# kwohlfahrt/collision

Measured on AMD Instinct MI355X. Metric: M spheres/sec end-to-end (bounds->Morton->radix sort->LBVH->refit->traversal), higher is better.
Workload: dtype f32 coords / u32 keys+ids; 1 GPU; BASELINE config 2: 1000000 uniform-random spheres, r=0.001, f32, RandomState(4), pair capacity 131072; spheres_total=1000000, group_size=256, parallelism=single

## Files before the change

collision_amd/csrc/bvh.hip:

```cpp
#include "col_common.h"
#include <math.h>

namespace {

constexpr u32 END = 0xFFFFFFFFu;

template <typename T> struct BTypes;
template <> struct BTypes<float> {
    typedef float4 V4;
    typedef uint32_t Bits;
    struct alignas(4) V3 { float x, y, z; };
};
template <> struct BTypes<double> {
    typedef double4 V4;
    typedef uint64_t Bits;
    struct alignas(8) V3 { double x, y, z; };
};

template <typename T> __device__ __forceinline__ u32 link_load(const T *bounds, uint64_t row) {
    typedef typename BTypes<T>::Bits Bits;
    return (u32) reinterpret_cast<const Bits *>(bounds)[row * 4 + 3];
}
template <typename T> __device__ __forceinline__ void link_store(T *bounds, uint64_t row, u32 v) {
    typedef typename BTypes<T>::Bits Bits;
// ... 923 lines not shown
    if (g_traverse_variant & 16) mode |= 8;
    if (g_traverse_variant & 256) mode |= 1;
    if (g_traverse_variant & 512) mode |= 2;
    if (g_traverse_variant & 16777216) mode |= 2048;
    if (g_traverse_variant & 33554432) mode |= 4096;
    constexpr int MAX_DEV = 16;
    static u64 *spread_dev[MAX_DEV] = {nullptr};
    static u32 *dyn_sched_dev[MAX_DEV] = {nullptr};
    int dev = 0;
    if (g_traverse_variant & (1024 | 8192)) {
        COL_HIP(hipGetDevice(&dev));
        if (dev < 0 || dev >= MAX_DEV) return COL_EINVAL;
    }
    u64 *&spread = spread_dev[dev];
    if (g_traverse_variant & 1024) {
        if (!spread && hipMalloc((void **)&spread, 8192 * 32 * 4) != hipSuccess) return COL_EINVAL;
        mode |= 16;
    }
    const bool off32 = (2ull * n - 1) * 8 * sizeof(T) < (1ull << 32) && !(g_traverse_variant & 64) && ((uintptr_t)bounds & 63) == 0;
    u32 *&dyn_sched = dyn_sched_dev[dev];
    if ((g_traverse_variant & 8192) && !sched && !st && !(mode & (32 | 64))) {
        if (!dyn_sched && hipMalloc((void **)&dyn_sched, 64) != hipSuccess) return COL_EINVAL;
        COL_HIP(hipMemsetAsync(dyn_sched, 0, 64, s));
        sched = dyn_sched;
    }
    if (sched && !st && !(g_traverse_variant & (16384 | 1 | 2 | 4 | 128 | 1024))) {
        mode |= 256;
        if (g_traverse_variant & 4194304) mode |= 128;
        if (g_traverse_variant & 8388608) mode |= 1024;
        if ((n <= COL_SPLIT_UNITS_UPTO || (g_traverse_variant & 65536)) && !(g_traverse_variant & 131072)) mode |= 512;
        if (off32 && (g_traverse_variant & 4096)) k_traverse<T, false, false, 1, false, true><<<g, t, 0, s>>>(pairs, counter, capacity, bd, n, (u64 *)sched, mode, NoGhost{}, n_dev, (g_traverse_variant & 2097152) ? nullptr : walk_order);
        else if (off32) k_traverse<T, false, false, 1><<<g, t, 0, s>>>(pairs, counter, capacity, bd, n, (u64 *)sched, mode, NoGhost{}, n_dev, (g_traverse_variant & 2097152) ? nullptr : walk_order);
        else k_traverse<T, false, false, 0><<<g, t, 0, s>>>(pairs, counter, capacity, bd, n, (u64 *)sched, mode, NoGhost{}, n_dev, (g_traverse_variant & 2097152) ? nullptr : walk_order);
        COL_LAUNCH_OK();
        return COL_OK;
    }
    if ((g_traverse_variant & 255) == 1) k_traverse_lane<T><<<g, t, 0, s>>>(pairs, counter, capacity, bd, n, 0);
    else if (st) k_traverse<T, true, false, 0><<<g, t, 0, s>>>(pairs, counter, capacity, bd, n, st, mode);
    else if (g_traverse_variant & 2) k_traverse<T, false, true, 0><<<g, t, 0, s>>>(pairs, counter, capacity, bd, n, st, mode);
    else if (off32 && (g_traverse_variant & 128)) k_traverse<T, false, false, 2><<<g, t, 0, s>>>(pairs, counter, capacity, bd, n, st, mode);
    else if (off32 && (g_traverse_variant & 4096)) k_traverse<T, false, false, 1, false, true><<<g, t, 0, s>>>(pairs, counter, capacity, bd, n, st, mode, NoGhost{}, n_dev);
    else if (off32) k_traverse<T, false, false, 1><<<g, t, 0, s>>>(pairs, counter, capacity, bd, n, (g_traverse_variant & 1024) ? spread : st, mode, NoGhost{}, n_dev);
    else k_traverse<T, false, false, 0><<<g, t, 0, s>>>(pairs, counter, capacity, bd, n, st, mode, NoGhost{}, n_dev);
    COL_LAUNCH_OK();
    return COL_OK;
}

__global__ __launch_bounds__(256) void k_pairs_compact(u32 *__restrict__ pairs, const ChunkHdr *__restrict__ hdr, u32 nholes) {
    __shared__ u32 s_start[512], s_len[512];
    __shared__ u32 s_low[513], s_fill[513];
    __shared__ u32 s_b[513], s_e[513];
    if (hdr->overflow) return;
    const u32 A = hdr->A, T = hdr->T, tid = threadIdx.x;
    if (A == T) return;
    __shared__ unsigned long long s_bits[1024];
    __shared__ u32 s_wpre[1024];
    __shared__ u32 s_ws2[4];
    for (u32 i = tid; i < 1024; i += 256) s_bits[i] = 0;
    for (u32 i = tid; i < 513; i += 256) { if (i < 512) { s_start[i] = A; s_len[i] = 0; } }
    __syncthreads();
    uint2 mine[2];
#pragma unroll
    for (int u = 0; u < 2; u++) {
        const u32 i = tid + 256 * u;
        mine[u] = i < nholes ? hdr->holes[i] : make_uint2(0u, 0u);
        if (mine[u].y) {
            const u32 c = mine[u].x / (u32)CHUNK_PAIRS;
            atomicOr(&s_bits[c >> 6], 1ull << (c & 63u));
        }
    }
    __syncthreads();
    {
        u32 pc[4], sum = 0;
#pragma unroll
        for (int u = 0; u < 4; u++) { pc[u] = (u32)__popcll(s_bits[4 * tid + u]); sum += pc[u]; }
        u32 total;
        u32 run = block_excl_scan<256>(sum, s_ws2, &total);
#pragma unroll
        for (int u = 0; u < 4; u++) { s_wpre[4 * tid + u] = run; run += pc[u]; }
    }
    __syncthreads();
#pragma unroll
    for (int u = 0; u < 2; u++)
        if (mine[u].y) {
            const u32 c = mine[u].x / (u32)CHUNK_PAIRS;
            const u32 rank = s_wpre[c >> 6] + (u32)__popcll(s_bits[c >> 6] & ((1ull << (c & 63u)) - 1ull));
            s_start[rank] = mine[u].x; s_len[rank] = mine[u].y;
        }
    __syncthreads();
    {
        __shared__ u32 s_ws[4];
        u32 lowc[2], highc[2], bb[2], ee[2];
#pragma unroll
        for (int u = 0; u < 2; u++) {
            const u32 i = 2 * tid + u;
            const u32 st = s_start[i], ln = s_len[i];
            bb[u] = ln ? (st > T ? st : T) : A;
            ee[u] = ln ? (st + ln > T ? st + ln : T) : A;
            lowc[u] = ln ? (st >= T ? 0u : (st + ln <= T ? ln : T - st)) : 0u;
            highc[u] = ee[u] - bb[u];
        }
        u32 total_low, total_high;
        const u32 plow = block_excl_scan<256>(lowc[0] + lowc[1], s_ws, &total_low);
        const u32 phigh = block_excl_scan<256>(highc[0] + highc[1], s_ws, &total_high);
#pragma unroll
        for (int u = 0; u < 2; u++) {
            const u32 i = 2 * tid + u;
            const u32 lo_before = plow + (u ? lowc[0] : 0u), hi_before = phigh + (u ? highc[0] : 0u);
            s_low[i] = lo_before;
            s_b[i] = bb[u]; s_e[i] = ee[u];
            s_fill[i] = (bb[u] - T) - hi_before;
        }
        if (tid == 0) {
            s_low[512] = total_low;
            s_fill[512] = (A - T) - total_high;
            s_b[512] = A; s_e[512] = A;
        }
    }
    __syncthreads();
    const u32 moves = s_low[512];
    constexpr int MV = 4;
    const u32 stride = gridDim.x * 256;
    for (u32 k0 = blockIdx.x * 256 + tid; k0 < moves; k0 += MV * stride) {
        u32 kk[MV], lo1[MV], lo2[MV];
#pragma unroll
        for (int u = 0; u < MV; u++) { kk[u] = min(k0 + u * stride, moves - 1u); lo1[u] = 0; lo2[u] = 0; }
#pragma unroll
        for (u32 step = 256; step; step >>= 1) {
#pragma unroll
            for (int u = 0; u < MV; u++) {
                if (s_low[lo1[u] + step] <= kk[u]) lo1[u] += step;
                if (s_fill[lo2[u] + step] <= kk[u]) lo2[u] += step;
            }
        }
        uint2 pr[MV];
        u32 dst[MV];
#pragma unroll
        for (int u = 0; u < MV; u++) {
            dst[u] = s_start[lo1[u]] + (kk[u] - s_low[lo1[u]]);
            const u32 src = kk[u] < s_fill[0] ? T + kk[u] : s_e[lo2[u]] + (kk[u] - s_fill[lo2[u]]);
            pr[u] = *reinterpret_cast<const uint2 *>(pairs + 2ull * src);
        }
#pragma unroll
        for (int u = 0; u < MV; u++)
            if (k0 + u * stride < moves) *reinterpret_cast<uint2 *>(pairs + 2ull * dst[u]) = pr[u];
    }
}

template <typename T>
int launch_traverse_chunked(void *stream, uint32_t *pairs, uint32_t *counter, uint32_t capacity, const void *bounds,
                            uint32_t n, void *scratch, const uint32_t *n_dev = nullptr, uint32_t *walk_order = nullptr,
                            bool hdr_cleared = false) {
    const bool split = (n <= COL_SPLIT_UNITS_UPTO || (g_traverse_variant & 65536)) && !(g_traverse_variant & 131072);
    const int dyn = (g_traverse_variant & 16384) ? 0 : (split ? 256 | 512 : 256) | ((g_traverse_variant & 4194304) ? 128 : 0) | ((g_traverse_variant & 8388608) ? 1024 : 0);
    const u32 npackets = (n + 63) / 64;
    u32 blocks = (u32)col_ceil_div(npackets, TW);
    if (blocks > 512) blocks = 512;
    dim3 g(blocks), t(TT);
    hipStream_t s = col_stream(stream);
    const T *bd = (const T *)bounds;
    ChunkHdr *hdr = (ChunkHdr *)scratch;
    if (!hdr_cleared) COL_HIP(hipMemsetAsync(hdr, 0, 64, s));
    k_traverse<T, false, false, 1><<<g, t, 0, s>>>(pairs, counter, capacity, bd, n, (u64 *)hdr, 32 | dyn, NoGhost{}, n_dev,
                                                   (dyn & 256) && !(g_traverse_variant & 2097152) ? walk_order : nullptr);
    COL_LAUNCH_OK();
    if (capacity) {
        k_pairs_compact<<<dim3(512), dim3(256), 0, s>>>(pairs, hdr, blocks);
        COL_LAUNCH_OK();
        k_traverse<T, false, false, 1><<<g, t, 0, s>>>(pairs, counter, capacity, bd, n, (u64 *)hdr, 64, NoGhost{}, n_dev);
        COL_LAUNCH_OK();
    }
    return COL_OK;
}

template <typename T>
int launch_ghost(void *stream, uint32_t *pairs, uint32_t *counter, uint32_t capacity, const void *bounds, uint32_t n,
                 const GhostArgs &ga, uint32_t max_ghosts, const uint32_t *n_dev) {
    const u32 npackets = (max_ghosts + 63) / 64;
    u32 blocks = (u32)col_ceil_div(npackets, TW);
    if (blocks > 512) blocks = 512;
    if (blocks == 0) return COL_OK;
    dim3 g(blocks), t(TT);
    hipStream_t s = col_stream(stream);
    const T *bd = (const T *)bounds;
    const bool off32 = (2ull * n - 1) * 8 * sizeof(T) < (1ull << 32) && !(g_traverse_variant & 64) && ((uintptr_t)bounds & 63) == 0;
    if (off32) k_traverse<T, false, false, 1, true><<<g, t, 0, s>>>(pairs, counter, capacity, bd, n, nullptr, 0, ga, n_dev);
    else k_traverse<T, false, false, 0, true><<<g, t, 0, s>>>(pairs, counter, capacity, bd, n, nullptr, 0, ga, n_dev);
    COL_LAUNCH_OK();
    return COL_OK;
}

}

extern "C" int col_traverse_ghost_packets(void *stream, uint32_t *pairs, uint32_t *counter, uint32_t capacity, const void *bounds,
                                          uint32_t n, int coord_bytes, const uint32_t *rec, const uint32_t *order,
                                          const uint32_t *count, uint32_t max_ghosts, const uint32_t *local_gids,
                                          const uint32_t *n_dev) {
    if (n == 0 || max_ghosts == 0) return COL_OK;
    const GhostArgs ga = {rec, order, count, local_gids};
    if (coord_bytes == 4) return launch_ghost<float>(stream, pairs, counter, capacity, bounds, n, ga, max_ghosts, n_dev);
    if (coord_bytes == 8) return launch_ghost<double>(stream, pairs, counter, capacity, bounds, n, ga, max_ghosts, n_dev);
    return COL_EINVAL;
}

extern "C" {

void col_debug_traverse(int variant) { g_traverse_variant = variant; }
int col_debug_walk_profile(uint32_t *out, uint32_t npackets) {
    if (npackets > COL_PROF_PACKETS) return COL_EINVAL;
    COL_HIP(hipDeviceSynchronize());
    COL_HIP(hipMemcpyFromSymbol(out, HIP_SYMBOL(g_walk_prof), 16ull * npackets));
    return COL_OK;
}

int col_bvh_build(void *stream, const uint32_t *codes, const uint32_t *ids, col_node *nodes, void *bounds,
                  uint32_t n, int coord_bytes) {
    if (n == 0) return COL_OK;
    if (n >= 0x80000000u) return COL_EINVAL;
    dim3 grid((unsigned)col_ceil_div(n, 256)), block(256);
    if (coord_bytes == 4) k_build<float><<<grid, block, 0, col_stream(stream)>>>(codes, ids, nodes, (float *)bounds, n);
    else if (coord_bytes == 8) k_build<double><<<grid, block, 0, col_stream(stream)>>>(codes, ids, nodes, (double *)bounds, n);
    else return COL_EINVAL;
    COL_LAUNCH_OK();
    return COL_OK;
}

int col_bvh_refit(void *stream, void *bounds, uint32_t *flags, const void *coords, const void *radii,
                  const col_node *nodes, uint32_t n, int coord_bytes) {
    if (n == 0) return COL_OK;
    if (coord_bytes != 4 && coord_bytes != 8) return COL_EINVAL;
    hipStream_t s = col_stream(stream);
    dim3 leaves((unsigned)col_ceil_div(n, 256)), inner((unsigned)col_ceil_div(n > 1 ? n - 1 : 1, 256)),
        all((unsigned)col_ceil_div(2ull * n - 1, 256)), block(256);
    int rounds = 16;
    for (uint32_t m = n; m > 1; m >>= 1) rounds++;
    uint32_t *progress = (n > (uint32_t)rounds + 1) ? flags + (n - 1) : nullptr;
    if (coord_bytes == 4) {
        k_refit_leaves<float><<<leaves, block, 0, s>>>((float *)bounds, flags, (const float *)coords, (const float *)radii, nodes, n);
        if (n > 1) {
            for (int r = 1; r <= rounds; r++) k_refit_sweep<float><<<inner, block, 0, s>>>((float *)bounds, flags, nodes, n, (u32)r, progress);
            k_refit_finish<float><<<all, block, 0, s>>>((float *)bounds, flags, nodes, n, progress ? progress + rounds : nullptr);
        }
    } else {
        k_refit_leaves<double><<<leaves, block, 0, s>>>((double *)bounds, flags, (const double *)coords, (const double *)radii, nodes, n);
        if (n > 1) {
            for (int r = 1; r <= rounds; r++) k_refit_sweep<double><<<inner, block, 0, s>>>((double *)bounds, flags, nodes, n, (u32)r, progress);
            k_refit_finish<double><<<all, block, 0, s>>>((double *)bounds, flags, nodes, n, progress ? progress + rounds : nullptr);
        }
    }
    COL_LAUNCH_OK();
    return COL_OK;
}

int col_traverse(void *stream, uint32_t *pairs, uint32_t *counter, uint32_t capacity, const col_node *nodes,
                 const void *bounds, uint32_t n, int coord_bytes) {
    (void)nodes;
    if (n < 2) return COL_OK;
    if (capacity > 0 && !pairs) return COL_EINVAL;
    if (coord_bytes == 4) return launch_traverse<float>(stream, pairs, counter, capacity, bounds, n, nullptr, 0);
    if (coord_bytes == 8) return launch_traverse<double>(stream, pairs, counter, capacity, bounds, n, nullptr, 0);
    return COL_EINVAL;
}

size_t col_traverse_chunked_scratch_bytes(void) { return sizeof(ChunkHdr); }

static int traverse_chunked_dev(void *stream, uint32_t *pairs, uint32_t *counter, uint32_t capacity, const col_node *nodes,
                                const void *bounds, uint32_t n, int coord_bytes, void *scratch, const uint32_t *n_dev,
                                uint32_t *walk_order = nullptr, bool hdr_cleared = false);
int col_traverse_chunked(void *stream, uint32_t *pairs, uint32_t *counter, uint32_t capacity, const col_node *nodes,
                         const void *bounds, uint32_t n, int coord_bytes, void *scratch) {
    return traverse_chunked_dev(stream, pairs, counter, capacity, nodes, bounds, n, coord_bytes, scratch, nullptr);
}
static int traverse_chunked_dev(void *stream, uint32_t *pairs, uint32_t *counter, uint32_t capacity, const col_node *nodes,
                                const void *bounds, uint32_t n, int coord_bytes, void *scratch, const uint32_t *n_dev,
                                uint32_t *walk_order, bool hdr_cleared) {
    const bool off32 = (coord_bytes == 4 || coord_bytes == 8) && (2ull * n - 1) * 8 * (unsigned)coord_bytes < (1ull << 32) &&
                       ((uintptr_t)bounds & 63) == 0;
    if (!off32 || !scratch || (g_traverse_variant & ~(16384 | 32768 | 65536 | 131072 | 2097152 | 4194304 | 8388608)))
    {
        if (n < 2) return COL_OK;
        if (capacity > 0 && !pairs) return COL_EINVAL;
        if (coord_bytes == 4) return launch_traverse<float>(stream, pairs, counter, capacity, bounds, n, nullptr, 0, nullptr, n_dev);
        if (coord_bytes == 8) return launch_traverse<double>(stream, pairs, counter, capacity, bounds, n, nullptr, 0, nullptr, n_dev);
        return COL_EINVAL;
    }
    if (n < 2) return COL_OK;
    if (capacity > 0 && !pairs) return COL_EINVAL;
    if (coord_bytes == 8) return launch_traverse_chunked<double>(stream, pairs, counter, capacity, bounds, n, scratch, n_dev, walk_order, hdr_cleared);
    return launch_traverse_chunked<float>(stream, pairs, counter, capacity, bounds, n, scratch, n_dev, walk_order, hdr_cleared);
}

int col_traverse_stats(void *stream, uint32_t *pairs, uint32_t *counter, uint32_t capacity, const void *bounds,
                       uint32_t n, int coord_bytes, uint64_t *stats, int mode) {
    if (n < 2) return COL_OK;
    if (coord_bytes == 4) return launch_traverse<float>(stream, pairs, counter, capacity, bounds, n, stats, mode);
    if (coord_bytes == 8) return launch_traverse<double>(stream, pairs, counter, capacity, bounds, n, stats, mode);
    return COL_EINVAL;
}

size_t col_collide_scratch_bytes(uint32_t n, uint32_t padded, int coord_bytes) {
    return 256  + col_reduce_scratch_bytes(coord_bytes == 8 ? COL_F64 : COL_F32, 4) +
           col_radix_scratch_bytes(padded, 4, 4) + col_lbvh_scratch_bytes(n, coord_bytes) +
           (size_t)n * 4 * coord_bytes  + sizeof(ChunkHdr) + 256  + 1024 +
           8 * ((size_t)n / 64 + 1) + 256 ;
}

int col_collide(void *stream, const void *coords, const void *radii, uint32_t n, uint32_t padded, int coord_bytes,
                uint32_t *codes0, uint32_t *codes1, uint32_t *ids0, uint32_t *ids1, col_node *nodes, void *bounds,
                uint32_t *flags, void *scratch, uint32_t *counter, uint32_t *pairs, uint32_t capacity) {
    return col_collide_plan(stream, coords, radii, n, padded, coord_bytes, codes0, codes1, ids0, ids1, nodes, bounds, flags,
                            scratch, counter, pairs, capacity, COL_SORT_LSD, nullptr);
}

int col_collide_plan(void *stream, const void *coords, const void *radii, uint32_t n, uint32_t padded, int coord_bytes,
                     uint32_t *codes0, uint32_t *codes1, uint32_t *ids0, uint32_t *ids1, col_node *nodes, void *bounds,
                     uint32_t *flags, void *scratch, uint32_t *counter, uint32_t *pairs, uint32_t capacity,
                     int sort_plan, uint32_t *oversize) {
    return col_collide_plan_partials(stream, coords, radii, n, padded, coord_bytes, codes0, codes1, ids0, ids1, nodes, bounds,
                                     flags, scratch, counter, pairs, capacity, sort_plan, oversize, nullptr, 0);
}

int col_collide_plan_partials(void *stream, const void *coords, const void *radii, uint32_t n, uint32_t padded, int coord_bytes,
                              uint32_t *codes0, uint32_t *codes1, uint32_t *ids0, uint32_t *ids1, col_node *nodes, void *bounds,
                              uint32_t *flags, void *scratch, uint32_t *counter, uint32_t *pairs, uint32_t capacity,
                              int sort_plan, uint32_t *oversize, const void *partials, uint32_t parts) {
    return col_collide_plan_dev(stream, coords, radii, n, padded, coord_bytes, codes0, codes1, ids0, ids1, nodes, bounds, flags, scratch,
                                counter, pairs, capacity, sort_plan, oversize, partials, parts, nullptr);
}

int col_collide_plan_dev(void *stream, const void *coords, const void *radii, uint32_t n, uint32_t padded, int coord_bytes,
                         uint32_t *codes0, uint32_t *codes1, uint32_t *ids0, uint32_t *ids1, col_node *nodes, void *bounds,
                         uint32_t *flags, void *scratch, uint32_t *counter, uint32_t *pairs, uint32_t capacity,
                         int sort_plan, uint32_t *oversize, const void *partials, uint32_t parts, const uint32_t *n_dev) {
    if (coord_bytes != 4 && coord_bytes != 8) return COL_EINVAL;
    if (n_dev && !partials) return COL_EINVAL;
    if (partials && (parts == 0 || parts > COL_MINMAX_PARTS)) return COL_EINVAL;
    if (padded < n || (capacity > 0 && !pairs)) return COL_EINVAL;
    if (!scratch) return COL_ENOSCRATCH;
    if (col_radix_tile_override_active()) return COL_EINVAL;
    hipStream_t s = col_stream(stream);
    if (n == 0) {
        COL_HIP(hipMemsetAsync(counter, 0, sizeof(uint32_t), s));
        return COL_OK;
    }
    (void)flags;
    char *p = (char *)scratch;
    void *range = p;           p += 256;
    void *red_scratch = p;     p += col_reduce_scratch_bytes(coord_bytes == 8 ? COL_F64 : COL_F32, 4);
    p = (char *)(((uintptr_t)p + 255) & ~(uintptr_t)255);
    void *sort_scratch = p;    p += col_radix_scratch_bytes(padded, 4, 4);
    p = (char *)(((uintptr_t)p + 255) & ~(uintptr_t)255);
    void *lbvh_scratch = p;    p += col_lbvh_scratch_bytes(n, coord_bytes);
    p = (char *)(((uintptr_t)p + 255) & ~(uintptr_t)255);
    void *packed = p;          p += (size_t)n * 4 * coord_bytes;
    p = (char *)(((uintptr_t)p + 255) & ~(uintptr_t)255);
    void *chunk_hdr = p;
    const bool chunked = (sort_plan & COL_TRAVERSE_CHUNKED) != 0;
    sort_plan &= 1;
    uint32_t *publish = oversize ? oversize + 2 : nullptr;
    int rc;
    uint32_t *report_word = nullptr;
    const uint32_t tile = col_radix_tile(padded, 4, 4);
    if (tile == 1024 || tile == 4096 || tile == 8192) {
        const bool msd = sort_plan == COL_SORT_MSD && padded <= COL_MSD_MAX_N;
        if (!partials) {
            if ((rc = col_minmax4_stage1(stream, coords, n, coord_bytes, red_scratch, &parts))) return rc;
            partials = red_scratch;
        }
        if ((rc = col_morton_tile(stream, coords, radii, partials, parts, n, padded, coord_bytes, codes0, ids0, packed,
                                  counter, (uint32_t *)sort_scratch, tile, (uint32_t)col_ceil_div(padded, tile), msd ? 22 : 0,
                                  publish, n_dev))) return rc;
        if (msd) rc = col_radix_sort_msd_dev(stream, codes0, codes1, ids0, ids1, padded, sort_scratch, oversize, n_dev);
        else rc = col_radix_sort_ex(stream, codes0, codes1, ids0, ids1, padded, 4, 4, sort_scratch, 0, 1);
        if (rc) return rc;
        if (!msd && oversize && padded <= COL_MSD_MAX_N) report_word = oversize + 1;
    } else {
        if (n_dev) return COL_EINVAL;
        if ((rc = col_reduce(stream, coords, n, coord_bytes == 8 ? COL_F64 : COL_F32, 4, COL_OP_MINMAX, red_scratch, range))) return rc;
        if ((rc = col_morton_ex(stream, coords, radii, range, n, padded, coord_bytes, codes0, ids0, packed, counter, publish))) return rc;
        if ((rc = col_radix_sort(stream, codes0, codes1, ids0, ids1, padded, 4, 4, sort_scratch, 0))) return rc;
    }
    uint32_t *sched = (!chunked && (n >= COL_DYNAMIC_PACKETS_FROM || (g_traverse_variant & 32768))) ? (uint32_t *)((char *)chunk_hdr + sizeof(ChunkHdr)) : nullptr;
    const int order_mode = chunked || col_lbvh_order_forced() ? 1 : 0;
    uint32_t *walk_order = n > 256 && (chunked || (sched && (n <= COL_DEAL_MAX_N || order_mode))) ? (uint32_t *)((char *)chunk_hdr + sizeof(ChunkHdr) + 256) : nullptr;
    if ((rc = col_lbvh_ex(stream, codes1, ids1, coords, radii, packed, nodes, bounds, lbvh_scratch, n, coord_bytes,
                          chunked ? (uint32_t *)chunk_hdr : sched, n_dev, walk_order, order_mode, chunked ? 16u : 8u, report_word, padded))) return rc;
    if (chunked) return traverse_chunked_dev(stream, pairs, counter, capacity, nodes, bounds, n, coord_bytes, chunk_hdr, n_dev, walk_order, true);
    if (n < 2) return COL_OK;
    if (coord_bytes == 4) return launch_traverse<float>(stream, pairs, counter, capacity, bounds, n, nullptr, 0, sched, n_dev, walk_order);
    return launch_traverse<double>(stream, pairs, counter, capacity, bounds, n, nullptr, 0, sched, n_dev, walk_order);
}

}
```

collision_amd/csrc/col_common.h:

```cpp
#pragma once
#include <hip/hip_runtime.h>
#include <stdint.h>
#include "../../include/collision_hip.h"
#include "../../include/collision_hip_debug.h"

#define COL_WAVE 64

#define COL_HIP(expr)                                  \
    do {                                               \
        hipError_t e_ = (expr);                        \
        if (e_ != hipSuccess) return (int)e_;          \
    } while (0)

#define COL_LAUNCH_OK()                                \
    do {                                               \
        hipError_t e_ = hipGetLastError();             \
        if (e_ != hipSuccess) return (int)e_;          \
    } while (0)

extern "C" int col_morton_ex(void *stream, const void *coords, const void *radii, const void *range, uint32_t n,
                             uint32_t padded, int coord_bytes, uint32_t *codes, uint32_t *ids, void *packed,
                             uint32_t *zero_word, uint32_t *publish);
extern "C" int col_lbvh_ex(void *stream, const uint32_t *codes, const uint32_t *ids, const void *coords, const void *radii,
                           const void *packed, col_node *nodes, void *bounds, void *scratch, uint32_t n, int coord_bytes,
                           uint32_t *zero8,
                           const uint32_t *n_dev,
                           uint32_t *walk_order,
                           int order_mode,
                           uint32_t nzero = 8,
                           uint32_t *report_word = nullptr,
                           uint32_t report_n = 0);
extern "C" int col_lbvh_order_forced(void);
extern "C" int col_radix_sort_msd_dev(void *stream, const uint32_t *keys, uint32_t *keys_out, const uint32_t *vals, uint32_t *vals_out,
                                      uint64_t n, void *scratch, uint32_t *oversize, const uint32_t *n_real_dev);

#define COL_MINMAX_PARTS 256
#define COL_REGION_BOXES 8
#define COL_MSD_SMALL_N 1900000u
#define COL_MSD_MAX_N 4050000u
extern "C" int col_minmax4_stage1(void *stream, const void *rows, uint64_t n, int coord_bytes, void *partials, uint32_t *parts);
extern "C" int col_minmax4_stage1_dev(void *stream, const void *rows, const uint32_t *n_dev, uint32_t n_max, int coord_bytes,
                                      void *partials, uint32_t *parts);
extern "C" int col_morton_tile(void *stream, const void *coords, const void *radii, const void *partials, uint32_t parts,
                               uint32_t n, uint32_t padded, int coord_bytes, uint32_t *codes, uint32_t *ids, void *packed,
                               uint32_t *zero_word, uint32_t *hist0, uint32_t tile, uint32_t nblocks, int hist_shift,
                               uint32_t *publish, const uint32_t *n_dev);
extern "C" int col_radix_sort_ex(void *stream, const void *keys, void *keys_out, const void *vals, void *vals_out,
                                 uint64_t n, int key_bytes, int val_bytes, void *scratch, int copy_back, int have_hist0);

extern "C" int col_traverse_ghost_packets(void *stream, uint32_t *pairs, uint32_t *counter, uint32_t capacity, const void *bounds,
                                          uint32_t n, int coord_bytes, const uint32_t *rec, const uint32_t *order,
                                          const uint32_t *count, uint32_t max_ghosts, const uint32_t *local_gids,
                                          const uint32_t *n_dev);
extern "C" int col_radix_sort_low_passes(void *stream, const uint32_t *keys, uint32_t *keys_out, const uint32_t *vals,
                                         uint32_t *vals_out, uint64_t n, void *scratch, int passes);
extern "C" int col_radix_bucket_report(void *stream, const uint32_t *sorted_codes, uint64_t n, uint32_t *word);
extern "C" int col_radix_tile_override_active(void);

static inline hipStream_t col_stream(void *s) { return (hipStream_t)s; }

static inline uint64_t col_ceil_div(uint64_t a, uint64_t b) { return (a + b - 1) / b; }

#ifdef __HIPCC__
typedef unsigned long long u64;
typedef unsigned int u32;
__device__ __forceinline__ void col_bucket_report_block(const u32 *__restrict__ sorted, u32 n, u32 *word, u32 *s_start) {
    const u32 d = threadIdx.x;
    const u32 want = d << 22;
    u32 lo = 0, hi = n;
    while (lo < hi) {
        const u32 mid = lo + ((hi - lo) >> 1);
        if (sorted[mid] < want) lo = mid + 1; else hi = mid;
    }
    s_start[d] = lo;
    if (d == 0) {
        u32 l2 = 0, h2 = n;
        while (l2 < h2) {
            const u32 mid = l2 + ((h2 - l2) >> 1);
            if (sorted[mid] < (1u << 30)) l2 = mid + 1; else h2 = mid;
        }
        s_start[256] = l2;
    }
    __syncthreads();
    u32 cnt = s_start[d + 1] - s_start[d];
#pragma unroll
    for (int o = COL_WAVE / 2; o > 0; o >>= 1) cnt = max(cnt, (u32)__shfl_xor((int)cnt, o, COL_WAVE));
    __syncthreads();
    if ((d & 63u) == 0) s_start[d >> 6] = cnt;
    __syncthreads();
    if (d == 0) {
        const u32 m = max(max(s_start[0], s_start[1]), max(s_start[2], s_start[3]));
        __hip_atomic_store(word, 0x80000000u | min(m, 0x7FFFFFFFu), __ATOMIC_RELAXED, __HIP_MEMORY_SCOPE_SYSTEM);
    }
}

__device__ __forceinline__ u32 lane_id() { return __lane_id(); }

__device__ __forceinline__ u32 count_of(u32 n, const u32 *__restrict__ n_dev) { return n_dev ? min(n, *n_dev) : n; }

__device__ __forceinline__ u32 mbcnt(u64 mask) {
    return __builtin_amdgcn_mbcnt_hi((u32)(mask >> 32), __builtin_amdgcn_mbcnt_lo((u32)mask, 0u));
}

__device__ __forceinline__ u32 wave_incl_scan(u32 v) {
    const u32 lane = lane_id();
#pragma unroll
    for (int o = 1; o < COL_WAVE; o <<= 1) {
        u32 t = __shfl_up(v, o, COL_WAVE);
        if (lane >= (u32)o) v += t;
    }
    return v;
}

__device__ __forceinline__ u32 wave_sum(u32 v) {
#pragma unroll
    for (int o = COL_WAVE / 2; o > 0; o >>= 1) v += __shfl_xor(v, o, COL_WAVE);
    return v;
}

template <int NT>
__device__ __forceinline__ u32 block_excl_scan(u32 v, u32 *warp_sums, u32 *total) {
    constexpr int NW = NT / COL_WAVE;
    const u32 lane = lane_id(), w = threadIdx.x / COL_WAVE;
    u32 incl = wave_incl_scan(v);
    if (lane == COL_WAVE - 1) warp_sums[w] = incl;
    __syncthreads();
    u32 base = 0, tot = 0;
#pragma unroll
    for (int i = 0; i < NW; i++) {
        u32 s = warp_sums[i];
        if ((u32)i < w) base += s;
        tot += s;
    }
    __syncthreads();
    *total = tot;
    return base + incl - v;
}
#define COL_LEAF_BLOCK 16u
#define COL_LINK_MARK 0x80000000u
#define COL_LEAF_BLOCK_MAX_N (1u << 27)
__device__ __forceinline__ u32 block_link(u32 lo, u32 hi) { return COL_LINK_MARK | (lo << 4) | (hi - lo); }
__device__ __forceinline__ u32 descend_link(u32 down, u32 leaf_start, bool marks) {
    return (marks && (down & COL_LINK_MARK)) ? leaf_start + ((down >> 4) & 0x7FFFFFFu) : down;
}
#define COL_DEAL_MAX_N 1310720u
#define COL_TRAV_WAVES 16u
#define COL_TRAV_FIRST_BATCHES 64
__device__ __forceinline__ void xcd_packet_range(u32 npackets, u32 x, u32 &p_lo, u32 &p_end) {
    const u32 ng = (npackets + COL_TRAV_WAVES - 1) / COL_TRAV_WAVES;
    p_lo = (u32)(((u64)ng * x) >> 3) * COL_TRAV_WAVES;
    p_end = min((u32)(((u64)ng * (x + 1)) >> 3) * COL_TRAV_WAVES, npackets);
}
__device__ __forceinline__ u32 expand_bits(u32 v) {
    v = (v * 0x00010001u) & 0xFF0000FFu;
    v = (v * 0x00000101u) & 0x0F00F00Fu;
    v = (v * 0x00000011u) & 0xC30C30C3u;
    v = (v * 0x00000005u) & 0x49249249u;
    return v;
}
template <typename T> __device__ __forceinline__ T tmax(T a, T b);
template <> __device__ __forceinline__ float tmax(float a, float b) { return fmaxf(a, b); }
template <> __device__ __forceinline__ double tmax(double a, double b) { return fmax(a, b); }
template <typename T> __device__ __forceinline__ T tmin(T a, T b);
template <> __device__ __forceinline__ float tmin(float a, float b) { return fminf(a, b); }
template <> __device__ __forceinline__ double tmin(double a, double b) { return fmin(a, b); }
template <typename T>
__device__ __forceinline__ u32 quantize(T p, T mn, T mx) {
    T t = (p - mn) / (mx - mn);
    t = t * (T)1023;
    t = tmin(tmax(t, (T)0), (T)1023);
    return (u32)t;
}
template <typename T>
__device__ __forceinline__ u32 morton30(T x, T y, T z, T mnx, T mny, T mnz, T mxx, T mxy, T mxz) {
    return (expand_bits(quantize(x, mnx, mxx)) << 2) + (expand_bits(quantize(y, mny, mxy)) << 1) +
           expand_bits(quantize(z, mnz, mxz));
}
#endif
```

collision_amd/csrc/lbvh.hip:

```cpp
#include "col_common.h"
#include <math.h>

namespace {

constexpr u32 END = 0xFFFFFFFFu;
constexpr int C = 256;
constexpr int LV = 9;

template <typename T> struct BT;
template <> struct BT<float> { typedef float4 V4; typedef uint32_t Bits; };
template <> struct BT<double> { typedef double4 V4; typedef uint64_t Bits; };

template <typename T> struct Box { T lo[3], hi[3]; };

template <typename T> __device__ __forceinline__ Box<T> box_empty() {
    Box<T> b;
#pragma unroll
    for (int a = 0; a < 3; a++) { b.lo[a] = (T)INFINITY; b.hi[a] = -(T)INFINITY; }
    return b;
}
__device__ __forceinline__ float hw_min(float a, float b) { float r; asm("v_min_f32 %0, %1, %2" : "=v"(r) : "v"(a), "v"(b)); return r; }
__device__ __forceinline__ float hw_max(float a, float b) { float r; asm("v_max_f32 %0, %1, %2" : "=v"(r) : "v"(a), "v"(b)); return r; }
__device__ __forceinline__ double hw_min(double a, double b) { double r; asm("v_min_f64 %0, %1, %2" : "=v"(r) : "v"(a), "v"(b)); return r; }
__device__ __forceinline__ double hw_max(double a, double b) { double r; asm("v_max_f64 %0, %1, %2" : "=v"(r) : "v"(a), "v"(b)); return r; }
// ... 462 lines not shown
        leaf.lo[0] = c.x - r; leaf.lo[1] = c.y - r; leaf.lo[2] = c.z - r;
        leaf.hi[0] = c.x + r; leaf.hi[1] = c.y + r; leaf.hi[2] = c.z + r;
        lds.leaf[0][tid] = c.x; lds.leaf[1][tid] = c.y; lds.leaf[2][tid] = c.z; lds.leaf[3][tid] = r;
    }

    Box<T> pre = leaf, suf = leaf;
    if constexpr (DPP_SCAN) {
        wave_prefix_union(pre);
        wave_suffix_union(suf);
    } else {
#pragma unroll
        for (int o = 1; o < COL_WAVE; o <<= 1) {
            const Box<T> up = box_shfl_up(pre, o), dn = box_shfl_down(suf, o);
            if (lane >= o) box_merge(pre, up);
            if (lane + o < COL_WAVE) box_merge(suf, dn);
        }
    }
    if (lane == COL_WAVE - 1) { for (int k = 0; k < 3; k++) { lds.wave_tot[0][w][k] = pre.lo[k]; lds.wave_tot[0][w][3 + k] = pre.hi[k]; } }
    if (lane == 0) { for (int k = 0; k < 3; k++) { lds.wave_tot[1][w][k] = suf.lo[k]; lds.wave_tot[1][w][3 + k] = suf.hi[k]; } }
    __syncthreads();
    for (int ww = 0; ww < C / COL_WAVE; ww++) {
        Box<T> t;
        for (int k = 0; k < 3; k++) { t.lo[k] = lds.wave_tot[ww < w ? 0 : 1][ww][k]; t.hi[k] = lds.wave_tot[ww < w ? 0 : 1][ww][3 + k]; }
        if (ww < w) box_merge(pre, t);
        if (ww > w) box_merge(suf, t);
    }

    if (valid) {
        LeafTail tail = {p, id};
        *reinterpret_cast<LeafTail *>(&nodes[leaf_start + p].right_edge) = tail;
        u32 skip_leaf = END;
        if (p + 1 < n) {
            if constexpr (FAST_DELTA && sizeof(I) == 4) {
                const u32 k = p + 1;
                if (k + 1 >= n) skip_leaf = (n - 1) + k;
                else if (tid + 1 < C) skip_leaf = lds.adj[tid + 2] > d_next ? k : (n - 1) + k;
                else skip_leaf = right_child_at(codes, k);
            } else skip_leaf = right_child_at(codes, p + 1);
        }
        record_store(bounds, (uint64_t)leaf_start + p, leaf, skip_leaf, id);
    }
    if (tid == 0)
        box_store(tab1, ((uint64_t)(chunk / C) * LV + 0) * C + (chunk % C), suf);
    if (p == n - 1 && n > (u32)C) box_store(partial, p, pre);
    if constexpr (CLIMB) {
        if (valid) {
            int l = tid, r = tid, my_split = 0;
            bool is_leaf = true;
            Box<T> box = leaf;
            for (;;) {
                const int dl = lds.adj[l], dr = lds.adj[r + 1];
                const bool right = dr > dl;
                if (!is_leaf) {
                    const int node = right ? r : l;
                    soa_put(lds.node, node, box);
                    lds.oe[node] = (unsigned char)(right ? l : r);
                    lds.split[node] = (unsigned char)my_split;
                }
                const int g = right ? r : l - 1;
                if ((dl & dr) < 0 || g < 0 || g >= C - 1) break;
                asm volatile("" ::: "memory");
                const u32 place = 16u * ((u32)g & 1u);
                const u32 old = (__hip_atomic_fetch_or(&lds.flags[g >> 1], ((u32)(right ? l : r) + 1u) << place, __ATOMIC_RELAXED, __HIP_MEMORY_SCOPE_WORKGROUP) >> place) & 0xFFFFu;
                asm volatile("" ::: "memory");
                if (old == 0) break;
                const int far = (int)old - 1;
                Box<T> sib;
                if (right) { sib = far == g + 1 ? leaf_get(lds.leaf, g + 1) : soa_get(lds.node, g + 1); r = far; }
                else { sib = far == g ? leaf_get(lds.leaf, g) : soa_get(lds.node, g); l = far; }
                box_merge(box, sib);
                my_split = g;
                is_leaf = false;
            }
        }
        __syncthreads();
    }
    auto search = [&](u32 t, u32 &j, u32 &gamma) {
        const u32 i = c0 + t, ci = codes.win[HALO + t];
        int dir, delta_min;
        if constexpr (FAST_DELTA && sizeof(I) == 4) {
            const int dn = lds.adj[t + 1], dp = lds.adj[t];
            dir = dn > dp ? 1 : -1;
            delta_min = min(dn, dp);
        } else {
            dir = delta(codes, i, ci, (I)i + 1) > delta(codes, i, ci, (I)i - 1) ? 1 : -1;
            delta_min = delta(codes, i, ci, (I)i - dir);
        }
        I len_max = 2;
        while (delta(codes, i, ci, (I)i + dir * len_max) > delta_min) len_max *= 2;
        I len = 0;
        for (I t2 = len_max / 2; t2 > 0; t2 /= 2)
            if (delta(codes, i, ci, (I)i + dir * (len + t2)) > delta_min) len += t2;
        j = (u32)((I)i + dir * len);
        const int delta_node = delta(codes, i, ci, (I)j);
        I s = 0, t2 = len;
        do {
            t2 = (t2 + 1) / 2;
            if (delta(codes, i, ci, (I)i + dir * (s + t2)) > delta_node) s += t2;
        } while (t2 > 1);
        gamma = dir > 0 ? (u32)(i + s) : (u32)(i - s - 1);
    };
    auto node_out = [&](u32 t, u32 j, u32 gamma, u32 &skip, u32 &child_a) {
        const u32 i = c0 + t;
        const u32 lo = min(i, j), hi = max(i, j);
        const bool a_leaf = lo == gamma, b_leaf = hi == gamma + 1;
        child_a = a_leaf ? leaf_start + gamma : gamma;
        const u32 child_b = b_leaf ? leaf_start + gamma + 1 : gamma + 1;
        InnerTail tail = {hi, child_a, child_b};
        *reinterpret_cast<InnerTail *>(&nodes[i].right_edge) = tail;
        if (!(dbg & 2)) { nodes[child_a].parent = i; nodes[child_b].parent = i; }
        other_end[i] = j;
        skip = END;
        if (hi + 1 < n) {
            if constexpr (FAST_DELTA && sizeof(I) == 4) {
                const u32 k = hi + 1;
                if (k + 1 >= n) skip = (n - 1) + k;
                else if (hi >= c0 && k < c0 + (u32)C) skip = lds.adj[k - c0 + 1] > lds.adj[hi - c0 + 1] ? k : (n - 1) + k;
                else {
                    const u32 ck = gcodes[k], cm = gcodes[k - 1u], cp = gcodes[k + 1u];
                    const u32 d_fwd = min(ffbh_raw(ck ^ cp), 32u + ffbh_raw(k ^ (k + 1u))), d_bwd = min(ffbh_raw(ck ^ cm), 32u + ffbh_raw(k ^ (k - 1u)));
                    skip = d_fwd > d_bwd ? k : (n - 1) + k;
                }
            } else skip = right_child_at(codes, hi + 1);
        }
    };
    auto record_out = [&](u32 i, u32 j, u32 skip, u32 child_a, const Box<T> &box) {
        const u32 lo = min(i, j), hi = max(i, j);
        u32 down = child_a;
        if (hi - lo < COL_LEAF_BLOCK && n <= COL_LEAF_BLOCK_MAX_N && block_k > (T)0) {
            const Box<T> first = leaf_get(lds.leaf, (int)(lo - c0));
            bool dense = true;
#pragma unroll
            for (int k = 0; k < 3; k++) dense = dense && (box.hi[k] - box.lo[k]) <= block_k * (first.hi[k] - first.lo[k]);
            if (dense) down = block_link(lo, hi);
        }
        record_store(bounds, (uint64_t)i, box, skip, down);
    };
    auto crossing_out = [&](u32 i, int dir) {
        box_store(partial, i, dir > 0 ? suf : pre);
        const u32 slot = atomicAdd(&lds.ncross, 1u);
        cross[(uint64_t)chunk * CROSS_CAP + (slot < CROSS_CAP - 1 ? slot : CROSS_CAP - 1)] = slot < CROSS_CAP - 1 ? i : CROSS_DENSE;
    };
    if constexpr (CLIMB) {
        const bool inner = p < leaf_start;
        const bool named = inner && lds.oe[tid] != (unsigned char)tid;
        u32 skip, child_a;
        if (named) {
            const u32 j = c0 + lds.oe[tid];
            node_out((u32)tid, j, c0 + lds.split[tid], skip, child_a);
            record_out(p, j, skip, child_a, soa_get(lds.node, tid));
        } else if (inner) crossing_out(p, d_next > d_prev ? 1 : -1);
        const u64 todo = __builtin_amdgcn_ballot_w64(inner && !named);
        if (todo == 0) return;
        const u32 cnt = (u32)__builtin_popcountll(todo);
        const u32 lpn_log = cnt <= 1 ? 6u : cnt <= 2 ? 5u : cnt <= 4 ? 4u : 3u, lpn = 1u << lpn_log, groups = 64u >> lpn_log;
        const u32 g = (u32)lane >> lpn_log, sub = (u32)lane & (lpn - 1u);
        auto group_count = [&](bool yes) -> I {
            u64 m = __builtin_amdgcn_ballot_w64(yes) >> (g << lpn_log);
            if (lpn < 64u) m &= (1ull << lpn) - 1ull;
            return (I)__builtin_popcountll(m);
        };
        for (u32 base = 0; base < cnt; base += groups) {
            const bool on = base + g < cnt;
            u64 m = todo;
            for (u32 b = 0; b < base + g && on; b++) m &= m - 1ull;
            const u32 t = on ? (u32)w * COL_WAVE + (u32)__builtin_ctzll(m) : (u32)tid;
            const u32 i = c0 + t, ci = codes.win[HALO + t];
            const int dn = lds.adj[t + 1], dp = lds.adj[t];
            const int dir = dn > dp ? 1 : -1, delta_min = min(dn, dp);
            auto yes_at = [&](I x, int thr) -> bool {
                const I jk = (I)i + dir * x;
                const bool inb = on && x > 0 && (u32)jk < n;
                const u32 o = (u32)(jk - codes.w0);
                const bool inwin = o < (u32)WIN;
                u32 cj;
                if (__builtin_amdgcn_ballot_w64(inb && !inwin) == 0) cj = codes.win[inwin ? o : 0u];
                else cj = inb ? (inwin ? codes.win[o] : gcodes[jk]) : 0u;
                const u32 d = min(ffbh_raw(ci ^ cj), 32u + ffbh_raw(i ^ (u32)jk));
                return inb && (int)d > thr;
            };
            I hi = 2;
            {
                bool more = on;
                int e0 = 1;
                while (__builtin_amdgcn_ballot_w64(more)) {
                    const int e = e0 + (int)sub;
                    const I x = (more && e < 31 && (1u << e) <= n) ? (I)(1u << e) : (I)0;
                    const I yes = group_count(yes_at(x, delta_min));
                    if (more) {
                        hi = (I)(1u << (e0 + yes));
                        more = yes == (I)lpn && e0 + (int)lpn < 31;
                        e0 += (int)lpn;
                    }
                }
            }
            auto run_end = [&](I lo, I hi, int thr) -> I {
                while (__builtin_amdgcn_ballot_w64(on && hi - lo > 1)) {
                    const bool act = on && hi - lo > 1;
                    const I step = (hi - lo + (I)lpn) / ((I)lpn + 1);
                    const I x = lo + ((I)sub + 1) * step;
                    const I yes = group_count(yes_at(act && x < hi ? x : (I)0, thr));
                    if (act) { lo += yes * step; hi = min(hi, lo + step); }
                }
                return lo;
            };
            const I len = run_end(hi / 2, hi, delta_min);
            const u32 j = (u32)((I)i + dir * len);
            const int delta_node = delta(codes, i, ci, (I)j);
            const I s = run_end((I)0, len, delta_node);
            const u32 gamma = dir > 0 ? (u32)(i + s) : (u32)(i - s - 1);
            if (on && sub == 0) {
                node_out(t, j, gamma, skip, child_a);
                links_store(bounds, (uint64_t)i, skip, child_a);
            }
        }
        return;
    }
    if (p >= leaf_start || (dbg & 4)) return;
    u32 j = 0, gamma = 0, skip, child_a;
    search((u32)tid, j, gamma);
    const u32 i = p;
    const u32 lo = min(i, j), hi = max(i, j);
    node_out((u32)tid, j, gamma, skip, child_a);
    if (dbg & 8) return;
    if (lo >= c0 && hi < c0 + C) {
        const bool a_leaf = lo == gamma, b_leaf = hi == gamma + 1;
        const int la = (int)(gamma - c0), lb = la + 1;
        Box<T> box;
        const int fa = a_leaf ? C : la, fb = b_leaf ? C : lb;
        for (bool done = false; !done;) {
            const u32 ra = __hip_atomic_load(&lds.flags[fa], __ATOMIC_RELAXED, __HIP_MEMORY_SCOPE_WORKGROUP);
            const u32 rb = __hip_atomic_load(&lds.flags[fb], __ATOMIC_RELAXED, __HIP_MEMORY_SCOPE_WORKGROUP);
            if (ra & rb) {
                __builtin_amdgcn_fence(__ATOMIC_ACQUIRE, "workgroup");
                box = a_leaf ? leaf_get(lds.leaf, la) : soa_get(lds.node, la);
                box_merge(box, b_leaf ? leaf_get(lds.leaf, lb) : soa_get(lds.node, lb));
                soa_put(lds.node, tid, box);
                __hip_atomic_store(&lds.flags[tid], 1u, __ATOMIC_RELEASE, __HIP_MEMORY_SCOPE_WORKGROUP);
                done = true;
            }
        }
        record_out(i, j, skip, child_a, box);
    } else {
        links_store(bounds, (uint64_t)i, skip, child_a);
        crossing_out(i, j > i ? 1 : -1);
    }
}

template <typename T>
__global__ __launch_bounds__(C) void k_group(T *__restrict__ tab, u32 count, T *__restrict__ next, u32 n_bound, const u32 *__restrict__ n_dev,
                                             int level) {
    if (n_dev) {
        u32 c = count_of(n_bound, n_dev);
        for (int k = 0; k <= level; k++) c = (c + C - 1) / C;
        count = min(count, c);
    }
    __shared__ Table<T> t;
    const int tid = threadIdx.x;
    const u32 g = blockIdx.x;
    const u32 e = g * C + tid;
    const uint64_t base = (uint64_t)g * LV * C;
    Box<T> b = e < count ? box_load(tab, base + tid) : box_empty<T>();
    if (e >= count) box_store(tab, base + tid, b);
    tab_put(t, 0, tid, b);
    tab_build(t, tid);
    for (int l = 1; l < LV; l++) box_store(tab, base + (uint64_t)l * C + tid, tab_get(t, l, tid));
    if (tid == 0 && next) box_store(next, ((uint64_t)(g / C) * LV + 0) * C + (g % C), tab_get(t, LV - 1, 0));
}

struct Tabs { void *t[3]; };

constexpr u32 LIN = 32;

template <typename T>
__device__ __forceinline__ void cross_node(T *__restrict__ bounds, const u32 *__restrict__ other_end, const T *__restrict__ partial,
                                           const Tabs &tabs, u32 i, int lin) {
    const u32 j = other_end[i];
    const u32 first = min(i, j), last = max(i, j);
    int64_t a = first / C, b = last / C;
    if (a == b) return;
    Box<T> box = box_load(partial, first);
    box_merge(box, box_load(partial, last));
    a += 1; b -= 1;
    for (int h = 0; h < 3 && a <= b; h++) {
        const T *tab = (const T *)tabs.t[h];
        if (h == lin) {
            for (int64_t e = a; e <= b; e++) box_merge(box, box_load(tab, (uint64_t)e));
            break;
        }
        const int64_t ga = a / C, gb = b / C;
        if (ga == gb) {
            box_merge(box, gtab_query(tab, (uint64_t)ga, (int)(a % C), (int)(b % C)));
            break;
        }
        box_merge(box, gtab_query(tab, (uint64_t)ga, (int)(a % C), C - 1));
        box_merge(box, gtab_query(tab, (uint64_t)gb, 0, (int)(b % C)));
        a = ga + 1; b = gb - 1;
    }
    T *row = bounds + 8ull * i;
    row[0] = box.lo[0]; row[1] = box.lo[1]; row[2] = box.lo[2];
    row[4] = box.hi[0]; row[5] = box.hi[1]; row[6] = box.hi[2];
}

template <typename T>
__global__ __launch_bounds__(256) void k_cross(T *__restrict__ bounds, const u32 *__restrict__ other_end,
                                               const T *__restrict__ partial, const u32 *__restrict__ cross, Tabs tabs, u32 n,
                                               u32 nchunks, int lin, u32 *__restrict__ zero8, const u32 *__restrict__ n_dev,
                                               u32 *__restrict__ walk_order, u32 cross_blocks, int order_mode, u32 nzero) {
    const u32 n_bound = n;
    if (n_dev) { n = count_of(n, n_dev); nchunks = min(nchunks, (n + (u32)C - 1) / (u32)C); }
    if (blockIdx.x >= cross_blocks) {
        order_packets(blockIdx.x - cross_blocks, n, n_bound, walk_order, order_mode);
        return;
    }
    const u32 t = blockIdx.x * 256 + threadIdx.x;
    if (zero8 && t < nzero) zero8[t] = 0;
    const u32 chunk = t / CROSS_CAP, slot = t % CROSS_CAP;
    if (chunk >= nchunks) return;
    if (cross[(uint64_t)chunk * CROSS_CAP + CROSS_CAP - 1] == CROSS_DENSE) {
        for (u32 k = slot; k < (u32)C; k += CROSS_CAP) {
            const u32 i = chunk * C + k;
            if (i + 1 < n) cross_node(bounds, other_end, partial, tabs, i, lin);
        }
        return;
    }
    const u32 i = cross[(uint64_t)chunk * CROSS_CAP + slot];
    if (i != END) cross_node(bounds, other_end, partial, tabs, i, lin);
}

int g_dbg = 0;
float g_block_k = 3.0f;
inline size_t align256(size_t x) { return (x + 255) & ~(size_t)255; }

struct Layout {
    size_t other_end, partial, cross, tab[3], total;
    u32 count[3];
};

Layout layout(uint32_t n, int coord_bytes) {
    Layout L;
    const size_t entry = 8 * (size_t)coord_bytes;
    size_t off = 0;
    L.other_end = off; off += align256((size_t)n * 4);
    L.partial = off;   off += align256((size_t)n * entry);
    u32 cnt = (u32)col_ceil_div(n, C);
    L.cross = off;     off += align256((size_t)cnt * CROSS_CAP * 4);
    for (int h = 0; h < 3; h++) {
        L.count[h] = cnt;
        const size_t groups = col_ceil_div(cnt, C);
        L.tab[h] = off; off += align256(groups * LV * C * entry);
        cnt = (u32)groups;
    }
    L.total = off;
    return L;
}

template <typename T>
int run(hipStream_t s, const u32 *codes, const u32 *ids, const T *coords, const T *radii, const T *packed,
        col_node *nodes, T *bounds, char *scratch, u32 n, u32 *zero8, const u32 *n_dev, u32 *walk_order, int order_mode,
        u32 nzero, u32 *report_word, u32 report_n) {
    const Layout L = layout(n, sizeof(T));
    u32 *other_end = (u32 *)(scratch + L.other_end);
    T *partial = (T *)(scratch + L.partial);
    u32 *cross = (u32 *)(scratch + L.cross);
    Tabs tabs;
    for (int h = 0; h < 3; h++) tabs.t[h] = scratch + L.tab[h];
    const u32 nchunks = L.count[0];
    bool ordered_by_chunk = false;
    if (g_dbg & ~(1024 | 2048 | 4096 | 8192 | 16384))
        k_chunk<T, true, int64_t><<<dim3(nchunks), dim3(C), 0, s>>>(codes, ids, coords, radii, packed, nodes, bounds, other_end, partial, cross,
                                                                    (T *)tabs.t[0], n, (T)g_block_k, n_dev, ChunkDiagOn{g_dbg & ~(1024 | 2048 | 4096 | 8192 | 16384)});
    else if (n < (1u << 30) && (g_dbg & 8192))
        k_chunk<T, false, int32_t, true, true><<<dim3(nchunks), dim3(C), 0, s>>>(codes, ids, coords, radii, packed, nodes, bounds, other_end, partial, cross,
                                                                                 (T *)tabs.t[0], n, (T)g_block_k, n_dev, ChunkDiagOff{});
    else if (n < (1u << 30) && !(g_dbg & 1024) && !((g_dbg & 2048) && sizeof(T) == 8))
    {
        k_chunk<T, false, int32_t, true, true, true><<<dim3(nchunks + (walk_order ? 8u * COL_ORDER_SLICES : 0u) + (report_word ? 1u : 0u)), dim3(C), (g_dbg & 16384) ? 24576 : 0, s>>>(
            codes, ids, coords, radii, packed, nodes, bounds, other_end, partial, cross, (T *)tabs.t[0], n, (T)g_block_k, n_dev, ChunkDiagOff{}, walk_order, order_mode,
            report_word, report_n);
        ordered_by_chunk = true;
        report_word = nullptr;
    }
    else if (n < (1u << 30) && !(g_dbg & 1024))
        k_chunk<T, false, int32_t, false, true><<<dim3(nchunks), dim3(C), 0, s>>>(codes, ids, coords, radii, packed, nodes, bounds, other_end, partial, cross,
                                                                                  (T *)tabs.t[0], n, (T)g_block_k, n_dev, ChunkDiagOff{});
    else if (n < (1u << 30))
        k_chunk<T, false, int32_t><<<dim3(nchunks), dim3(C), 0, s>>>(codes, ids, coords, radii, packed, nodes, bounds, other_end, partial, cross,
                                                                     (T *)tabs.t[0], n, (T)g_block_k, n_dev, ChunkDiagOff{});
    else
        k_chunk<T, false, int64_t><<<dim3(nchunks), dim3(C), 0, s>>>(codes, ids, coords, radii, packed, nodes, bounds, other_end, partial, cross,
                                                                     (T *)tabs.t[0], n, (T)g_block_k, n_dev, ChunkDiagOff{});
    COL_LAUNCH_OK();
    if (report_word) {
        const int rc = col_radix_bucket_report((void *)s, codes, report_n, report_word);
        if (rc) return rc;
    }
    if (nchunks < 2) {
        if (zero8) COL_HIP(hipMemsetAsync(zero8, 0, nzero * sizeof(u32), s));
        return COL_OK;
    }
    int lin = -1;
    for (int h = 0; h < 3; h++) {
        if (h > 0 && L.count[h] <= LIN) { lin = h; break; }
        const u32 groups = (u32)col_ceil_div(L.count[h], C);
        k_group<T><<<dim3(groups), dim3(C), 0, s>>>((T *)tabs.t[h], L.count[h], h + 1 < 3 ? (T *)tabs.t[h + 1] : nullptr, n, n_dev, h);
        COL_LAUNCH_OK();
        if (groups < 2) break;
    }
    const unsigned cross_blocks = (unsigned)col_ceil_div((uint64_t)nchunks * CROSS_CAP, 256);
    k_cross<T><<<dim3(cross_blocks + (walk_order && !ordered_by_chunk ? 8u * COL_ORDER_SLICES : 0u)), dim3(256), 0, s>>>(bounds, other_end, partial, cross, tabs, n, nchunks, lin, zero8,
                                                                                                          n_dev, walk_order, cross_blocks, order_mode, nzero);
    COL_LAUNCH_OK();
    return COL_OK;
}

}

extern "C" {

void col_debug_lbvh(int mode) { g_dbg = mode; }
int col_lbvh_order_forced(void) { return (g_dbg & 4096) ? 1 : 0; }
void col_debug_leaf_blocks(float k) { g_block_k = k; }

size_t col_lbvh_scratch_bytes(uint32_t n, int coord_bytes) { return layout(n, coord_bytes).total + 256; }

int col_lbvh_ex(void *stream, const uint32_t *codes, const uint32_t *ids, const void *coords, const void *radii,
                const void *packed, col_node *nodes, void *bounds, void *scratch, uint32_t n, int coord_bytes, uint32_t *zero8,
                const uint32_t *n_dev, uint32_t *walk_order, int order_mode, uint32_t nzero, uint32_t *report_word, uint32_t report_n) {
    if (n == 0) return COL_OK;
    if (n >= 0x80000000u || nzero > 256u) return COL_EINVAL;
    if (!scratch) return COL_ENOSCRATCH;
    if (coord_bytes == 4)
        return run<float>(col_stream(stream), codes, ids, (const float *)coords, (const float *)radii, (const float *)packed,
                          nodes, (float *)bounds, (char *)scratch, n, zero8, n_dev, walk_order, order_mode, nzero, report_word, report_n);
    if (coord_bytes == 8)
        return run<double>(col_stream(stream), codes, ids, (const double *)coords, (const double *)radii,
                           (const double *)packed, nodes, (double *)bounds, (char *)scratch, n, zero8, n_dev, walk_order, order_mode, nzero, report_word, report_n);
    return COL_EINVAL;
}

int col_lbvh(void *stream, const uint32_t *codes, const uint32_t *ids, const void *coords, const void *radii,
             col_node *nodes, void *bounds, void *scratch, uint32_t n, int coord_bytes) {
    return col_lbvh_ex(stream, codes, ids, coords, radii, nullptr, nodes, bounds, scratch, n, coord_bytes, nullptr, nullptr, nullptr, 0);
}

}
```

collision_amd/csrc/morton.hip:

```cpp
#include "col_common.h"

namespace {


template <typename T> struct alignas(4 * sizeof(T)) Vec4 { T x, y, z, w; };
template <> struct alignas(16) Vec4<double> { double x, y, z, w; };

__device__ __forceinline__ void publish_count(u32 *publish, u32 count) {
    if (publish) __hip_atomic_store(publish, 0x80000000u | (count < 0x7FFFFFFFu ? count : 0x7FFFFFFFu), __ATOMIC_RELAXED, __HIP_MEMORY_SCOPE_SYSTEM);
}

template <typename T>
__global__ __launch_bounds__(256) void k_morton(const Vec4<T> *__restrict__ coords,
                                                 const Vec4<T> *__restrict__ range, u32 n, u32 padded,
                                                 u32 *__restrict__ codes, u32 *__restrict__ ids,
                                                 const T *__restrict__ radii, Vec4<T> *__restrict__ packed,
                                                 u32 *__restrict__ zero_word, u32 *publish) {
    const u32 i = blockIdx.x * 256 + threadIdx.x;
    if (i == 0 && zero_word) {
        publish_count(publish, *zero_word);
        *zero_word = 0;
    }
    if (i >= padded) return;
    u32 code = 0xFFFFFFFFu;
    if (i < n) {
        const Vec4<T> mn = range[0], mx = range[1];
        const Vec4<T> c = coords[i];
        if (packed) {
            Vec4<T> pr = c;
            pr.w = radii[i];
            packed[i] = pr;
        }
        code = (expand_bits(quantize(c.x, mn.x, mx.x)) << 2) + (expand_bits(quantize(c.y, mn.y, mx.y)) << 1) +
               expand_bits(quantize(c.z, mn.z, mx.z));
    }
    codes[i] = code;
    if (ids) ids[i] = i;
}

constexpr int MT_ROWS = 4;
template <typename T, int NT, int HALVES>
__global__ __launch_bounds__(NT) void k_morton_tile(const Vec4<T> *__restrict__ coords, const T *__restrict__ partials,
                                                     u32 parts, u32 n_bound, u32 padded, u32 *__restrict__ codes,
                                                     u32 *__restrict__ ids, const T *__restrict__ radii,
                                                     Vec4<T> *__restrict__ packed, u32 *__restrict__ zero_word,
                                                     u32 *__restrict__ hist0, u32 nblocks, int hist_shift, u32 *publish,
                                                     const u32 *__restrict__ n_dev) {
    constexpr int TILE = NT * MT_ROWS * HALVES, NW = NT / 64;
    const u32 n = count_of(n_bound, n_dev);
    __shared__ T s_fold[NW][8];
    __shared__ u32 s_hist[256];
    const u32 tid = threadIdx.x, lane = tid & 63u, w = tid >> 6;
    if (blockIdx.x == 0 && tid == 0 && zero_word) {
        publish_count(publish, *zero_word);
        *zero_word = 0;
    }
    if (tid < 256) s_hist[tid] = 0;
    Vec4<T> c[MT_ROWS];
    T rad[MT_ROWS];
#pragma unroll
    for (int k = 0; k < MT_ROWS; k++) {
        const u32 i = blockIdx.x * TILE + k * NT + tid;
        if (i < n) {
            c[k] = coords[i];
            if (packed) rad[k] = radii[i];
        }
    }
    T acc[8];
#pragma unroll
    for (int k = 0; k < 4; k++) { acc[k] = (T)INFINITY; acc[4 + k] = -(T)INFINITY; }
    for (u32 i = tid; i < parts; i += NT) {
        const T *q = partials + (size_t)i * 8;
#pragma unroll
        for (int k = 0; k < 4; k++) {
            acc[k] = q[k] < acc[k] ? q[k] : acc[k];
            acc[4 + k] = q[4 + k] > acc[4 + k] ? q[4 + k] : acc[4 + k];
        }
    }
#pragma unroll
    for (int o = 32; o > 0; o >>= 1) {
#pragma unroll
        for (int k = 0; k < 4; k++) {
            const T lo = __shfl_xor(acc[k], o, 64), hi = __shfl_xor(acc[4 + k], o, 64);
            acc[k] = lo < acc[k] ? lo : acc[k];
            acc[4 + k] = hi > acc[4 + k] ? hi : acc[4 + k];
        }
    }
    if (lane == 0) {
#pragma unroll
        for (int k = 0; k < 8; k++) s_fold[w][k] = acc[k];
    }
    __syncthreads();
    Vec4<T> mn, mx;
    {
        T r[8];
#pragma unroll
        for (int k = 0; k < 8; k++) r[k] = s_fold[0][k];
        for (int ww = 1; ww < NW; ww++) {
#pragma unroll
            for (int k = 0; k < 4; k++) {
                r[k] = s_fold[ww][k] < r[k] ? s_fold[ww][k] : r[k];
                r[4 + k] = s_fold[ww][4 + k] > r[4 + k] ? s_fold[ww][4 + k] : r[4 + k];
            }
        }
        mn.x = r[0]; mn.y = r[1]; mn.z = r[2]; mn.w = r[3];
        mx.x = r[4]; mx.y = r[5]; mx.z = r[6]; mx.w = r[7];
    }
#pragma unroll
    for (int h = 0; h < HALVES; h++) {
        if (h > 0) {
#pragma unroll
            for (int k = 0; k < MT_ROWS; k++) {
                const u32 i = blockIdx.x * TILE + (h * MT_ROWS + k) * NT + tid;
                if (i < n) {
                    c[k] = coords[i];
                    if (packed) rad[k] = radii[i];
                }
            }
        }
#pragma unroll
        for (int k = 0; k < MT_ROWS; k++) {
            const u32 i = blockIdx.x * TILE + (h * MT_ROWS + k) * NT + tid;
            if (i >= padded) continue;
            u32 code = 0xFFFFFFFFu;
            if (i < n) {
                if (packed) {
                    Vec4<T> pr = c[k];
                    pr.w = rad[k];
                    packed[i] = pr;
                }
                code = (expand_bits(quantize(c[k].x, mn.x, mx.x)) << 2) + (expand_bits(quantize(c[k].y, mn.y, mx.y)) << 1) +
                       expand_bits(quantize(c[k].z, mn.z, mx.z));
            }
            codes[i] = code;
            if (ids) ids[i] = i;
            atomicAdd(&s_hist[(code >> hist_shift) & 255u], 1u);
        }
    }
    __syncthreads();
    if (tid < 256) hist0[(uint64_t)tid * nblocks + blockIdx.x] = s_hist[tid];
}

template <typename T>
int launch_morton_tile(hipStream_t s, u32 tile, const void *coords, const void *radii, const void *partials, uint32_t parts,
                       uint32_t n, uint32_t padded, uint32_t *codes, uint32_t *ids, void *packed, uint32_t *zero_word,
                       uint32_t *hist0, uint32_t nblocks, int hist_shift, uint32_t *publish, const uint32_t *n_dev) {
    dim3 grid(nblocks);
    if (tile == 1024)
        k_morton_tile<T, 256, 1><<<grid, dim3(256), 0, s>>>((const Vec4<T> *)coords, (const T *)partials, parts, n, padded, codes, ids,
                                                             (const T *)radii, (Vec4<T> *)packed, zero_word, hist0, nblocks, hist_shift, publish, n_dev);
    else if (tile == 4096)
        k_morton_tile<T, 1024, 1><<<grid, dim3(1024), 0, s>>>((const Vec4<T> *)coords, (const T *)partials, parts, n, padded, codes, ids,
                                                               (const T *)radii, (Vec4<T> *)packed, zero_word, hist0, nblocks, hist_shift, publish, n_dev);
    else
        k_morton_tile<T, 1024, 2><<<grid, dim3(1024), 0, s>>>((const Vec4<T> *)coords, (const T *)partials, parts, n, padded, codes, ids,
                                                               (const T *)radii, (Vec4<T> *)packed, zero_word, hist0, nblocks, hist_shift, publish, n_dev);
    COL_LAUNCH_OK();
    return COL_OK;
}

}

extern "C" {

int col_morton_tile(void *stream, const void *coords, const void *radii, const void *partials, uint32_t parts,
                    uint32_t n, uint32_t padded, int coord_bytes, uint32_t *codes, uint32_t *ids, void *packed,
                    uint32_t *zero_word, uint32_t *hist0, uint32_t tile, uint32_t nblocks, int hist_shift, uint32_t *publish,
                    const uint32_t *n_dev) {
    if (padded < n || parts == 0 || !hist0 || hist_shift < 0 || hist_shift > 24) return COL_EINVAL;
    if (tile != 1024 && tile != 4096 && tile != 8192) return COL_EINVAL;
    if (padded == 0) return COL_OK;
    if (packed && !radii) return COL_EINVAL;
    if (nblocks != (uint32_t)col_ceil_div(padded, tile)) return COL_EINVAL;
    if (coord_bytes == 4)
        return launch_morton_tile<float>(col_stream(stream), tile, coords, radii, partials, parts, n, padded, codes, ids, packed,
                                         zero_word, hist0, nblocks, hist_shift, publish, n_dev);
    if (coord_bytes == 8)
        return launch_morton_tile<double>(col_stream(stream), tile, coords, radii, partials, parts, n, padded, codes, ids, packed,
                                          zero_word, hist0, nblocks, hist_shift, publish, n_dev);
    return COL_EINVAL;
}

int col_morton_ex(void *stream, const void *coords, const void *radii, const void *range, uint32_t n, uint32_t padded,
                  int coord_bytes, uint32_t *codes, uint32_t *ids, void *packed, uint32_t *zero_word, uint32_t *publish) {
    if (padded < n) return COL_EINVAL;
    if (padded == 0) return COL_OK;
    if (packed && !radii) return COL_EINVAL;
    dim3 grid((unsigned)col_ceil_div(padded, 256)), block(256);
    if (coord_bytes == 4)
        k_morton<float><<<grid, block, 0, col_stream(stream)>>>((const Vec4<float> *)coords, (const Vec4<float> *)range, n, padded,
                                                                codes, ids, (const float *)radii, (Vec4<float> *)packed, zero_word, publish);
    else if (coord_bytes == 8)
        k_morton<double><<<grid, block, 0, col_stream(stream)>>>((const Vec4<double> *)coords, (const Vec4<double> *)range, n,
                                                                 padded, codes, ids, (const double *)radii, (Vec4<double> *)packed,
                                                                 zero_word, publish);
    else
        return COL_EINVAL;
    COL_LAUNCH_OK();
    return COL_OK;
}

int col_morton(void *stream, const void *coords, const void *range, uint32_t n, uint32_t padded, int coord_bytes,
               uint32_t *codes, uint32_t *ids) {
    return col_morton_ex(stream, coords, nullptr, range, n, padded, coord_bytes, codes, ids, nullptr, nullptr, nullptr);
}

}
```

collision_amd/csrc/radix.hip:

```cpp
#include "col_common.h"
#include <algorithm>

namespace {

constexpr int RT = 256;
constexpr int RDIG = 256;
constexpr int BS_SHIFT_REPORT = 22;
constexpr int IT_BIG = 16, IT_SMALL = 4, IT_HUGE = 32;
constexpr int NT_BIG = 512, NT_MID = 256, NT_SMALL = 256, NT_HUGE = 512;
#ifndef COL_SCATTER_KEYS_FIRST
#define COL_SCATTER_KEYS_FIRST 0
#endif
constexpr uint64_t SMALL_N = 1u << 20, BIG_N_DEFAULT = 8u << 20, HUGE_N = 32u << 20;
constexpr int HG = 16;

template <int B> struct Val;
template <> struct Val<4> { typedef uint32_t T; };
template <> struct Val<8> { typedef uint2 T; };
template <> struct Val<16> { typedef uint4 T; };
struct alignas(16) V32 { uint4 a, b; };
template <> struct Val<32> { typedef V32 T; };

template <typename K> __device__ __forceinline__ u32 digit_of(K key, int shift) { return (u32)(key >> shift) & (RDIG - 1); }

__device__ unsigned long long g_stamp[8];
struct DiagOff {};
struct DiagOn { int mode; };
template <bool DIAG> struct DiagArg { typedef DiagOff T; };
template <> struct DiagArg<true> { typedef DiagOn T; };
__device__ __forceinline__ constexpr int diag_mode(DiagOff) { return 0; }
__device__ __forceinline__ int diag_mode(DiagOn d) { return d.mode; }
#define STAMP(slot)                                                              \
    if (DIAG && (dbg & 32) && threadIdx.x == 0) {                                \
        const unsigned long long t_ = __builtin_amdgcn_s_memtime();              \
        atomicAdd(&g_stamp[slot], t_ - t_prev);                                  \
        t_prev = t_;                                                             \
    }

__device__ __forceinline__ u64 match8(u32 d) {
    u32 m[8];
    u64 bal[8];
#pragma unroll
    for (int b = 0; b < 8; b++) {
        m[b] = (u32)__builtin_amdgcn_sbfe(d, b, 1);
        asm("" : "+v"(m[b]));
    }
#pragma unroll
    for (int b = 0; b < 8; b++) bal[b] = __builtin_amdgcn_ballot_w64(m[b] != 0);
    u32 dlo = 0, dhi = 0;
#pragma unroll
    for (int b = 0; b < 8; b++) {
        dlo = __builtin_amdgcn_bitop3_b32(dlo, (u32)bal[b], m[b], 0xF6);
        dhi = __builtin_amdgcn_bitop3_b32(dhi, (u32)(bal[b] >> 32), m[b], 0xF6);
    }
    return ~(((u64)dhi << 32) | dlo);
}

constexpr int HC = 16;
template <typename K, int TILE>
__global__ __launch_bounds__(RT) __attribute__((amdgpu_num_sgpr(80))) void k_hist(const K *__restrict__ keys, uint64_t n, u32 nblocks, u32 g,
                                             int shift, u32 *__restrict__ hist) {
    constexpr int IT = TILE / RT;
    constexpr int VEC = 16 / sizeof(K);
    constexpr int NV = IT / VEC;
    __shared__ __attribute__((aligned(16))) u32 col[RDIG * HC];
    __shared__ u32 h[HG * RDIG];
    typedef u32 v4u __attribute__((ext_vector_type(4)));
    const u32 tid = threadIdx.x, c = tid & (HC - 1);
#pragma unroll
    for (int j = 0; j < HC / 4; j++) *reinterpret_cast<v4u *>(col + tid * HC + 4 * j) = v4u{0, 0, 0, 0};
    __syncthreads();
    const u32 b0 = blockIdx.x * g;
    const u32 cnt = min(g, nblocks - b0);
    const u32 m = cnt && (uint64_t)(b0 + cnt) * TILE > n ? cnt - 1 : cnt;
    auto issue = [&](v4u (&dst)[NV], uint64_t base) {
#pragma unroll
        for (int k = 0; k < NV; k++)
            asm volatile("global_load_dwordx4 %0, %1, off" : "=v"(dst[k]) : "v"(keys + base + ((uint64_t)k * RT + tid) * VEC) : "memory");
    };
    auto arrived = [&](v4u (&dst)[NV]) {
#pragma unroll
        for (int k = 0; k < NV; k++) asm volatile("s_waitcnt vmcnt(0)" : "+v"(dst[k])::"memory");
    };
    auto fold = [&](u32 t) {
        __syncthreads();
        u32 sum = 0;
#pragma unroll
        for (int j = 0; j < HC / 4; j++) {
            v4u *p = reinterpret_cast<v4u *>(col + tid * HC + 4 * ((j + (tid >> 2)) & (HC / 4 - 1)));
            const v4u v = *p;
            sum += v.x + v.y + v.z + v.w;
            *p = v4u{0, 0, 0, 0};
        }
        h[t * RDIG + tid] = sum;
        __syncthreads();
    };
    auto count = [&](const v4u (&src)[NV]) {
#pragma unroll
        for (int k = 0; k < NV; k++) {
            K kk[VEC];
            *reinterpret_cast<v4u *>(kk) = src[k];
#pragma unroll
            for (int j = 0; j < VEC; j++) atomicAdd(&col[digit_of(kk[j], shift) * HC + c], 1u);
        }
    };
    if (m) {
        v4u q[NV], qn[NV];
        issue(q, (uint64_t)b0 * TILE);
        arrived(q);
        for (u32 t = 0; t + 1 < m; t++) {
            if constexpr (NV <= 8) {
                issue(qn, (uint64_t)(b0 + t + 1) * TILE);
                count(q);
                fold(t);
                arrived(qn);
#pragma unroll
                for (int k = 0; k < NV; k++) q[k] = qn[k];
            } else {
                count(q);
                fold(t);
                issue(q, (uint64_t)(b0 + t + 1) * TILE);
                arrived(q);
            }
        }
        count(q);
        fold(m - 1);
    }
    if (m < cnt) {
        const uint64_t base = (uint64_t)(b0 + m) * TILE;
        for (int k = 0; k < IT; k++) {
            const uint64_t i = base + (uint64_t)k * RT + tid;
            if (i < n) atomicAdd(&col[digit_of(keys[i], shift) * HC + c], 1u);
        }
        fold(m);
    }
    u32 *row = hist + (uint64_t)tid * nblocks + b0;
    for (u32 t = 0; t < cnt; t++) row[t] = h[t * RDIG + tid];
}

template <int SCOPE, typename X> __device__ __forceinline__ void st_scope(X *p, X v) {
    if constexpr (sizeof(X) == 4) __hip_atomic_store(reinterpret_cast<u32 *>(p), *reinterpret_cast<u32 *>(&v), __ATOMIC_RELAXED, SCOPE);
    else if constexpr (sizeof(X) == 8) __hip_atomic_store(reinterpret_cast<u64 *>(p), *reinterpret_cast<u64 *>(&v), __ATOMIC_RELAXED, SCOPE);
    else *p = v;
}

template <bool NARROW> struct CntType { typedef u32 T; };
template <> struct CntType<true> { typedef uint16_t T; };
template <typename K, int VB, int IT, int NT, bool DIAG>
__global__ __launch_bounds__(NT) void k_scatter(const K *__restrict__ keys_in, K *__restrict__ keys_out,
                                                const void *__restrict__ vals_in_, void *__restrict__ vals_out_,
                                                uint64_t n, u32 nblocks, int shift,
                                                const u32 *__restrict__ offsets, typename DiagArg<DIAG>::T diag) {
    const int dbg = diag_mode(diag);
    constexpr int TILE = NT * IT;
    constexpr int NW = NT / COL_WAVE;
    constexpr bool HAS_V = VB > 0;
    constexpr bool V_LDS = VB == 4 || VB == 8;
    typedef typename Val<(VB > 0 ? VB : 4)>::T V;
    __shared__ __attribute__((aligned(16))) K s_keys[TILE];
    __shared__ __attribute__((aligned(16))) V s_vals[V_LDS ? TILE : 1];
    typedef typename CntType<(NT > 512)>::T CNT;
    __shared__ CNT s_cnt[NW][RDIG];
    __shared__ u32 s_goff[RDIG];
    __shared__ u32 s_ws[NW];
    __shared__ u32 s_dstart[DIAG ? RDIG : 1];

    const V *vals_in = reinterpret_cast<const V *>(vals_in_);
    V *vals_out = reinterpret_cast<V *>(vals_out_);
    const u32 tid = threadIdx.x, lane = tid & (COL_WAVE - 1), w = tid / COL_WAVE;
    u32 b = blockIdx.x;
    if (DIAG && (dbg & (1 << 22)) && nblocks % (8u << ((dbg >> 24) & 7)) == 0) {
        const u32 G = 1u << ((dbg >> 24) & 7), x = b % 8, j = b / 8;
        b = ((j / G) * 8 + x) * G + (j % G);
    } else if (!(dbg & 4)) {
        const u32 q = nblocks / 8, r = nblocks % 8, xcd = b % 8;
        b = (xcd < r ? xcd * (q + 1) : r * (q + 1) + (xcd - r) * q) + b / 8;
    }
    const uint64_t tile_base = (uint64_t)b * TILE;
    const u32 valid = (u32)min((uint64_t)TILE, n - tile_base);

    unsigned long long t_prev = (DIAG && (dbg & 32)) ? __builtin_amdgcn_s_memtime() : 0ull;
    (void)t_prev;
    if (DIAG && (dbg & (1 << 27))) __builtin_amdgcn_s_setprio(3);
    const u32 my_offset = tid < RDIG ? offsets[(uint64_t)tid * nblocks + b] : 0u;
    for (u32 i = tid; i < NW * RDIG; i += NT) (&s_cnt[0][0])[i] = (CNT)0;

    const u32 wbase = w * (COL_WAVE * IT) + lane;
    K key[IT];
    V val[V_LDS ? IT : 1];
    constexpr int KV = 16 / sizeof(K);
    constexpr int VV = 16 / sizeof(V);
    constexpr int NVQ = V_LDS ? IT / VV : 0;
    typedef u32 v4u __attribute__((ext_vector_type(4)));
    v4u vq[V_LDS ? IT / VV : 1];
    V *vstage = s_vals + w * (COL_WAVE * IT);
    const bool full = valid == (u32)TILE && !(dbg & 8);
    if (full) {
        K *stage = s_keys + w * (COL_WAVE * IT);
        const K *src = keys_in + tile_base + w * (COL_WAVE * IT);
        const V *vsrc = vals_in + tile_base + w * (COL_WAVE * IT);
        v4u kq[IT / KV];
        if (dbg & 64) {
#pragma unroll
            for (int j = 0; j < IT / KV; j++)
                asm volatile("global_load_dwordx4 %0, %1, off nt" : "=v"(kq[j]) : "v"(src + j * (COL_WAVE * KV) + lane * KV) : "memory");
            if (V_LDS) {
#pragma unroll
                for (int j = 0; j < IT / VV; j++)
                    asm volatile("global_load_dwordx4 %0, %1, off nt" : "=v"(vq[j]) : "v"(vsrc + j * (COL_WAVE * VV) + lane * VV) : "memory");
            }
        } else {
#pragma unroll
            for (int j = 0; j < IT / KV; j++)
                asm volatile("global_load_dwordx4 %0, %1, off" : "=v"(kq[j]) : "v"(src + j * (COL_WAVE * KV) + lane * KV) : "memory");
            if (V_LDS) {
#pragma unroll
                for (int j = 0; j < IT / VV; j++)
                    asm volatile("global_load_dwordx4 %0, %1, off" : "=v"(vq[j]) : "v"(vsrc + j * (COL_WAVE * VV) + lane * VV) : "memory");
            }
        }
#pragma unroll
        for (int j = 0; j < IT / KV; j++) asm volatile("s_waitcnt vmcnt(%1)" : "+v"(kq[j]) : "n"(COL_SCATTER_KEYS_FIRST ? NVQ : 0) : "memory");
#pragma unroll
        for (int j = 0; j < IT / KV; j++)
            *reinterpret_cast<v4u *>(stage + j * (COL_WAVE * KV) + lane * KV) = kq[j];
        __builtin_amdgcn_wave_barrier();
#pragma unroll
        for (int k = 0; k < IT; k++) key[k] = stage[k * COL_WAVE + lane];
    } else {
#pragma unroll
        for (int k = 0; k < IT; k++) {
            const u32 li = wbase + k * COL_WAVE;
            key[k] = li < valid ? keys_in[tile_base + li] : (K)~(K)0;
        }
        if (V_LDS) {
#pragma unroll
            for (int k = 0; k < IT; k++) {
                const u32 li = wbase + k * COL_WAVE;
                if (li < valid) val[k] = vals_in[tile_base + li];
            }
        }
#pragma unroll
        for (int k = 0; k < IT; k++) asm volatile("" : "+v"(key[k]));
        if (V_LDS) {
#pragma unroll
            for (int k = 0; k < IT; k++) {
                u32 *words = reinterpret_cast<u32 *>(&val[k]);
#pragma unroll
                for (int c = 0; c < (int)(sizeof(V) / 4); c++) asm volatile("" : "+v"(words[c]));
            }
        }
    }
    if (DIAG && (dbg & (1 << 27))) __builtin_amdgcn_s_setprio(0);
    __syncthreads();
    STAMP(0)
    if (DIAG && (dbg & (1 << 28))) __builtin_amdgcn_s_setprio(3);

    const bool norank = DIAG && (dbg & 65536);
    u32 pos[IT];
    const bool atomrank = DIAG && sizeof(CNT) == 4 && (dbg & (1 << 21));
    if (atomrank) {
        if constexpr (sizeof(CNT) == 4) {
#pragma unroll
            for (int k = 0; k < IT; k++) pos[k] = atomicAdd(reinterpret_cast<u32 *>(&s_cnt[w][digit_of(key[k], shift)]), 1u);
        }
    } else if (!norank) {
#pragma unroll
    for (int k = 0; k < IT; k++) {
        const u32 d = digit_of(key[k], shift);
        const u64 peers = match8(d);
        const u32 below = mbcnt(peers);
        const u32 prev = s_cnt[w][d];
        if (below == 0) s_cnt[w][d] = (CNT)(prev + (u32)__popcll(peers));
        pos[k] = prev + below;
    }
    }
    if (V_LDS && full) {
#pragma unroll
        for (int j = 0; j < IT / VV; j++) asm volatile("s_waitcnt vmcnt(0)" : "+v"(vq[j])::"memory");
#pragma unroll
        for (int j = 0; j < IT / VV; j++)
            *reinterpret_cast<v4u *>(vstage + j * (COL_WAVE * VV) + lane * VV) = vq[j];
        __builtin_amdgcn_wave_barrier();
#pragma unroll
        for (int k = 0; k < IT; k++) val[k] = vstage[k * COL_WAVE + lane];
    }
    if (DIAG && (dbg & (1 << 28))) __builtin_amdgcn_s_setprio(0);
    __syncthreads();
    STAMP(1)

    if (norank) {
#pragma unroll
        for (int k = 0; k < IT; k++) pos[k] = wbase + k * COL_WAVE;
        u32 cnt = 0;
        if (tid < RDIG) {
            const uint64_t flat = (uint64_t)tid * nblocks + b;
            cnt = (flat + 1 < (uint64_t)RDIG * nblocks ? offsets[flat + 1] : (u32)n) - my_offset;
        }
        u32 total;
        const u32 dstart = block_excl_scan<NT>(cnt, s_ws, &total);
        if (tid < RDIG) {
            s_goff[tid] = my_offset - dstart;
            for (int i = 0; i < NW; i++) s_cnt[i][tid] = 0;
            if (DIAG) s_dstart[tid] = dstart;
        }
    } else
    {
        u32 c[NW], tot = 0;
        if (tid < RDIG) {
#pragma unroll
            for (int i = 0; i < NW; i++) { c[i] = s_cnt[i][tid]; tot += c[i]; }
        }
        u32 total;
        const u32 dstart = block_excl_scan<NT>(tot, s_ws, &total);
        if (tid < RDIG) {
            u32 run = dstart;
#pragma unroll
            for (int i = 0; i < NW; i++) { s_cnt[i][tid] = (CNT)run; run += c[i]; }
            s_goff[tid] = my_offset - dstart;
            if (DIAG) s_dstart[tid] = dstart;
        }
    }
    __syncthreads();
    STAMP(2)

#pragma unroll
    for (int k = 0; k < IT; k++) {
        const u32 d = digit_of(key[k], shift);
        pos[k] += s_cnt[w][d];
        s_keys[pos[k]] = key[k];
        if (V_LDS) s_vals[pos[k]] = val[k];
    }
    if (HAS_V && !V_LDS) {
#pragma unroll
        for (int k = 0; k < IT; k++) {
            const u32 li = wbase + k * COL_WAVE;
            if (li < valid) vals_out[s_goff[digit_of(key[k], shift)] + pos[k]] = vals_in[tile_base + li];
        }
    }
    __syncthreads();
    STAMP(3)

    if (DIAG && (dbg & (1 << 23))) __builtin_amdgcn_s_setprio(3);
#pragma unroll
    for (int k = 0; k < IT; k++) {
        const u32 i = k * NT + tid;
        if (DIAG && (dbg & (1 << 29)) && k) __builtin_amdgcn_s_sleep(2);
        if (i < valid) {
            const K kk = s_keys[i];
            u32 g = s_goff[digit_of(kk, shift)] + i;
            if (DIAG) {
                if (dbg & 2) g = (u32)tile_base + i;
                if (dbg & 32768) g &= (1u << 20) - 1;
                if (dbg & 8192) {
                    const u32 d = digit_of(kk, shift);
                    g = (u32)(((u64)d * nblocks + b) * 32 + min(i - s_dstart[d], 31u));
                }
            }
            if (DIAG && (dbg & 16384)) {
                if constexpr (V_LDS && sizeof(K) == 4 && VB == 4)
                    reinterpret_cast<uint2 *>(keys_out)[g] = make_uint2(kk, s_vals[i]);
            } else if (DIAG && (dbg & 384)) {
                if (dbg & 128) {
                    st_scope<__HIP_MEMORY_SCOPE_SYSTEM>(&keys_out[g], kk);
                    if (V_LDS) st_scope<__HIP_MEMORY_SCOPE_SYSTEM>(&vals_out[g], s_vals[i]);
                } else {
                    st_scope<__HIP_MEMORY_SCOPE_AGENT>(&keys_out[g], kk);
                    if (V_LDS) st_scope<__HIP_MEMORY_SCOPE_AGENT>(&vals_out[g], s_vals[i]);
                }
            } else {
                keys_out[g] = kk;
                if (V_LDS) vals_out[g] = s_vals[i];
            }
        }
    }
    if (dbg & 32) { __builtin_amdgcn_s_waitcnt(0); }
    STAMP(4)
}


template <bool RAGGED>
__global__ __launch_bounds__(NT_HUGE, 4) void k_scatter_huge(const u32 *__restrict__ keys_in, u32 *__restrict__ keys_out,
                                                             uint64_t n, u32 nblocks, u32 first_tile, int shift,
                                                             const u32 *__restrict__ offsets) {
    constexpr int NT = NT_HUGE, IT = IT_HUGE, TILE = NT * IT, NW = NT / COL_WAVE, SLICE = COL_WAVE * IT;
    __shared__ __attribute__((aligned(16))) u32 s_img[TILE];
    __shared__ u32 s_cnt[NW][RDIG];
    __shared__ u32 s_goff[RDIG];
    __shared__ u32 s_ws[NW];
    typedef u32 v4u __attribute__((ext_vector_type(4)));
    const u32 tid = threadIdx.x, lane = tid & (COL_WAVE - 1), w = tid / COL_WAVE;
    u32 b = blockIdx.x;
    if (!RAGGED) {
        const u32 q = gridDim.x / 8, r = gridDim.x % 8, xcd = b % 8;
        b = (xcd < r ? xcd * (q + 1) : r * (q + 1) + (xcd - r) * q) + b / 8;
    }
    b += first_tile;
    const uint64_t tile_base = (uint64_t)b * TILE;
    const u32 valid = RAGGED ? (u32)(n - tile_base) : (u32)TILE;
    const u32 my_offset = tid < RDIG ? offsets[(uint64_t)tid * nblocks + b] : 0u;
    for (u32 i = lane; i < RDIG; i += COL_WAVE) s_cnt[w][i] = 0;
    u32 *stage = s_img + w * SLICE;
    v4u kq[IT / 4];
    const u32 e0 = w * SLICE + lane * 4;
    if (!RAGGED) {
#pragma unroll
        for (int j = 0; j < IT / 4; j++)
            asm volatile("global_load_dwordx4 %0, %1, off" : "=v"(kq[j]) : "v"(keys_in + tile_base + e0 + j * (COL_WAVE * 4)) : "memory");
#pragma unroll
        for (int j = 0; j < IT / 4; j++) asm volatile("s_waitcnt vmcnt(0)" : "+v"(kq[j])::"memory");
    } else {
#pragma unroll
        for (int j = 0; j < IT / 4; j++) {
            const u32 e = e0 + j * (COL_WAVE * 4);
            for (int c = 0; c < 4; c++) kq[j][c] = e + c < valid ? keys_in[tile_base + e + c] : 0xFFFFFFFFu;
        }
    }
#pragma unroll
    for (int j = 0; j < IT / 4; j++) *reinterpret_cast<v4u *>(stage + j * (COL_WAVE * 4) + lane * 4) = kq[j];
    __builtin_amdgcn_wave_barrier();

    u32 pos[IT];
#pragma unroll
    for (int k = 0; k < IT; k++) {
        const u32 d = digit_of(stage[k * COL_WAVE + lane], shift);
        const u64 peers = match8(d);
        const u32 below = mbcnt(peers);
        const u32 prev = s_cnt[w][d];
        if (below == 0) s_cnt[w][d] = prev + (u32)__popcll(peers);
        pos[k] = prev + below;
    }
    __syncthreads();
    {
        u32 c[NW], tot = 0;
        if (tid < RDIG) {
#pragma unroll
            for (int i = 0; i < NW; i++) { c[i] = s_cnt[i][tid]; tot += c[i]; }
        }
        u32 total;
        const u32 dstart = block_excl_scan<NT>(tot, s_ws, &total);
        if (tid < RDIG) {
            u32 run = dstart;
#pragma unroll
            for (int i = 0; i < NW; i++) { s_cnt[i][tid] = run; run += c[i]; }
            s_goff[tid] = my_offset - dstart;
        }
    }
    __syncthreads();
    {
        u32 key[IT];
#pragma unroll
        for (int k = 0; k < IT; k++) {
            key[k] = stage[k * COL_WAVE + lane];
            pos[k] += s_cnt[w][digit_of(key[k], shift)];
        }
        __syncthreads();
#pragma unroll
        for (int k = 0; k < IT; k++) s_img[pos[k]] = key[k];
    }
    __syncthreads();
#pragma unroll
    for (int k = 0; k < IT; k++) {
        const u32 i = k * NT + tid;
        if (i < valid) {
            const u32 kk = s_img[i];
            keys_out[s_goff[digit_of(kk, shift)] + i] = kk;
        }
    }
}

constexpr int BS_NT = 1024, BS_NW = BS_NT / COL_WAVE;
constexpr int BS_SHIFT = 22;

template <int BS_IT> struct BucketLds {
    u32 keys[BS_NT * BS_IT];
    u32 vals[BS_NT * BS_IT];
    u32 cnt[BS_NW][RDIG];
    u32 base[RDIG];
    u32 ws[BS_NW];
};

template <int BS_IT>
__device__ __forceinline__ void bucket_rank(BucketLds<BS_IT> &lds, const u32 (&key)[BS_IT], u32 (&pos)[BS_IT], u32 m, int shift,
                                            u32 w, u32 tid, u32 row_len) {
    for (u32 i = tid; i < BS_NW * RDIG; i += BS_NT) (&lds.cnt[0][0])[i] = 0;
    __syncthreads();
#pragma unroll
    for (int k = 0; k < BS_IT; k++) {
        pos[k] = 0;
        if ((u32)k * COL_WAVE >= row_len || w * row_len + k * COL_WAVE >= m) continue;
        const u32 d = digit_of(key[k], shift);
        const u64 peers = match8(d);
        const u32 below = mbcnt(peers);
        const u32 prev = lds.cnt[w][d];
        if (below == 0) lds.cnt[w][d] = prev + (u32)__popcll(peers);
        pos[k] = prev + below;
    }
    __syncthreads();
}

template <int BS_IT>
__global__ __launch_bounds__(BS_NT) void k_bucket_sort(u32 *__restrict__ k_a, u32 *__restrict__ v_a, u32 *__restrict__ k_b,
                                                        u32 *__restrict__ v_b, u32 n, const u32 *__restrict__ offsets,
                                                        u32 nblocks, u32 *oversize, const u32 *__restrict__ n_real_dev) {
    constexpr u32 BS_CAP = BS_NT * BS_IT;
    constexpr int BS_ROW = COL_WAVE * BS_IT;
    __shared__ BucketLds<BS_IT> lds;
    const u32 tid = threadIdx.x, lane = tid & (COL_WAVE - 1);
    const u32 w = (u32)__builtin_amdgcn_readfirstlane((int)(tid / COL_WAVE));
    const u32 d = blockIdx.x;
    const u32 start = offsets[(uint64_t)d * nblocks], end = d + 1 < RDIG ? offsets[(uint64_t)(d + 1) * nblocks] : n;
    u32 pads = 0;
    if (n_real_dev) {
        const u32 n_real = min(n, *n_real_dev), all = n - n_real, per = (all + RDIG - 1) / RDIG;
        for (u32 i = threadIdx.x; i < per; i += BS_NT) {
            const u32 j = n_real + d * per + i;
            if (j < n) { k_b[j] = 0xFFFFFFFFu; v_b[j] = j; }
        }
        if (d == RDIG - 1) pads = min(end - start, all);
    }
    const u32 S = end - start - pads;
    if (S == 0) return;
    u32 key[BS_IT], val[BS_IT], pos[BS_IT];

    if (S <= BS_CAP) {
        const u32 L = ((S + BS_NW - 1) / BS_NW + COL_WAVE - 1) & ~(u32)(COL_WAVE - 1);
#pragma unroll
        for (int k = 0; k < BS_IT; k++) {
            const u32 p = w * L + k * COL_WAVE + lane;
            const bool ok = (u32)k * COL_WAVE < L && p < S;
            key[k] = ok ? k_a[start + p] : 0xFFFFFFFFu;
            val[k] = ok ? v_a[start + p] : 0u;
        }
        for (int shift = 0; shift < BS_SHIFT; shift += 8) {
            bucket_rank<BS_IT>(lds, key, pos, S, shift, w, tid, L);
            {
                u32 c[BS_NW], tot = 0;
                if (tid < RDIG) {
#pragma unroll
                    for (int i = 0; i < BS_NW; i++) { c[i] = lds.cnt[i][tid]; tot += c[i]; }
                }
                u32 total;
                const u32 dstart = block_excl_scan<BS_NT>(tot, lds.ws, &total);
                if (tid < RDIG) {
                    u32 run = dstart;
#pragma unroll
                    for (int i = 0; i < BS_NW; i++) { lds.cnt[i][tid] = run; run += c[i]; }
                }
            }
            __syncthreads();
#pragma unroll
            for (int k = 0; k < BS_IT; k++) {
                if ((u32)k * COL_WAVE >= L || w * L + k * COL_WAVE >= S) continue;
                const u32 q = pos[k] + lds.cnt[w][digit_of(key[k], shift)];
                lds.keys[q] = key[k];
                lds.vals[q] = val[k];
            }
            __syncthreads();
#pragma unroll
            for (int k = 0; k < BS_IT; k++) {
                const u32 p = w * L + k * COL_WAVE + lane;
                if ((u32)k * COL_WAVE >= L || w * L + k * COL_WAVE >= S) continue;
                key[k] = p < S ? lds.keys[p] : 0xFFFFFFFFu;
                val[k] = p < S ? lds.vals[p] : 0u;
            }
        }
#pragma unroll
        for (int k = 0; k < BS_IT; k++) {
            const u32 p = w * L + k * COL_WAVE + lane;
            if ((u32)k * COL_WAVE < L && p < S) { k_b[start + p] = key[k]; v_b[start + p] = val[k]; }
        }
        return;
    }

    if (tid == 0 && oversize) *oversize = S;
    int pass = 0;
    for (int shift = 0; shift < BS_SHIFT; shift += 8, pass++) {
        const u32 *sk = ((pass & 1) ? k_b : k_a) + start, *sv = ((pass & 1) ? v_b : v_a) + start;
        u32 *dk = ((pass & 1) ? k_a : k_b) + start, *dv = ((pass & 1) ? v_a : v_b) + start;
        if (tid < RDIG) lds.base[tid] = 0;
        __syncthreads();
        for (u32 i = tid; i < S; i += BS_NT) atomicAdd(&lds.base[digit_of(sk[i], shift)], 1u);
        __syncthreads();
        {
            u32 total;
            const u32 mine = tid < RDIG ? lds.base[tid] : 0u;
            const u32 ex = block_excl_scan<BS_NT>(mine, lds.ws, &total);
            if (tid < RDIG) lds.base[tid] = ex;
        }
        __syncthreads();
        for (u32 c0 = 0; c0 < S; c0 += BS_CAP) {
            const u32 m = min(BS_CAP, S - c0);
#pragma unroll
            for (int k = 0; k < BS_IT; k++) {
                const u32 p = w * BS_ROW + k * COL_WAVE + lane;
                key[k] = p < m ? sk[c0 + p] : 0xFFFFFFFFu;
                val[k] = p < m ? sv[c0 + p] : 0u;
            }
            bucket_rank<BS_IT>(lds, key, pos, m, shift, w, tid, (u32)BS_ROW);
            if (tid < RDIG) {
                u32 run = lds.base[tid];
#pragma unroll
                for (int i = 0; i < BS_NW; i++) { const u32 c = lds.cnt[i][tid]; lds.cnt[i][tid] = run; run += c; }
                if (tid == RDIG - 1) {
                    const u32 ranked = ((m + COL_WAVE - 1) / COL_WAVE) * COL_WAVE;
                    run -= ranked - m;
                }
                lds.base[tid] = run;
            }
            __syncthreads();
// ... 88 lines not shown
        const u32 d = (u32)(kk >> shift) & (nd - 1);
        const u32 dst = loff[d] + i - lstart[d];
        keys_out[dst] = kk;
        if (vals && vals_out) for (u32 q = 0; q < vb; q++) vals_out[(uint64_t)dst * vb + q] = vals[src * vb + q];
    }
}

int g_radix_dbg = 0;
int g_radix_tile_override = 0;
int g_radix_wide_block = 0;
uint64_t g_big_n = BIG_N_DEFAULT;
#define BIG_N g_big_n
inline size_t align256(size_t x) { return (x + 255) & ~(size_t)255; }
inline bool huge_ok(int key_bytes, int val_bytes) { return key_bytes == 4 && val_bytes == 0; }
inline u32 tile_auto(uint64_t n, int key_bytes, int val_bytes) {
    u32 t = n < SMALL_N ? (u32)(NT_SMALL * IT_SMALL) : n < BIG_N ? (u32)(NT_MID * IT_BIG) : (u32)(NT_BIG * IT_BIG);
    if (n >= HUGE_N && huge_ok(key_bytes, val_bytes)) t = (u32)(NT_HUGE * IT_HUGE);
    if (key_bytes == 8 && t > (u32)(NT_MID * IT_BIG)) t = (u32)(NT_MID * IT_BIG);
    return t;
}
inline u32 tile_for(uint64_t n, int key_bytes, int val_bytes) {
    if (!g_radix_tile_override) return tile_auto(n, key_bytes, val_bytes);
    u32 t = (u32)g_radix_tile_override;
    if (t > (u32)(NT_BIG * IT_BIG) && !huge_ok(key_bytes, val_bytes)) t = (u32)(NT_BIG * IT_BIG);
    if (key_bytes == 8 && t > (u32)(NT_MID * IT_BIG)) t = (u32)(NT_MID * IT_BIG);
    return t;
}
inline u32 tiles_of(uint64_t n, int key_bytes, int val_bytes) { return (u32)col_ceil_div(n, tile_for(n, key_bytes, val_bytes)); }
inline size_t max_tiles_upto(uint64_t n, int key_bytes) {
    if (n == 0) return 1;
    size_t m = col_ceil_div(n < SMALL_N ? n : SMALL_N - 1, NT_SMALL * IT_SMALL);
    if (n >= SMALL_N) {
        const uint64_t top = (key_bytes == 8 || n < BIG_N) ? n : BIG_N - 1;
        m = std::max(m, (size_t)col_ceil_div(top, NT_MID * IT_BIG));
    }
    if (n >= BIG_N && key_bytes != 8) m = std::max(m, (size_t)col_ceil_div(n, NT_BIG * IT_BIG));
    if (g_radix_tile_override) m = std::max(m, (size_t)col_ceil_div(n, NT_SMALL * IT_SMALL));
    return m;
}

inline u32 hist_group(u32 nblocks) {
    u32 g = HG;
    while (g > 1 && nblocks / g < 1024) g >>= 1;
    return g;
}

template <typename K>
int launch_hist(hipStream_t s, const void *keys, uint64_t n, int val_bytes, int pass, u32 *hist) {
    const u32 tile = tile_for(n, (int)sizeof(K), val_bytes);
    const u32 nb = tiles_of(n, (int)sizeof(K), val_bytes), g = hist_group(nb);
    dim3 grid((unsigned)col_ceil_div(nb, g)), block(RT);
    const K *k = (const K *)keys;
    if (tile == (u32)(NT_SMALL * IT_SMALL)) k_hist<K, NT_SMALL * IT_SMALL><<<grid, block, 0, s>>>(k, n, nb, g, pass * 8, hist);
    else if (tile == (u32)(NT_MID * IT_BIG)) k_hist<K, NT_MID * IT_BIG><<<grid, block, 0, s>>>(k, n, nb, g, pass * 8, hist);
    else if (tile == (u32)(NT_BIG * IT_BIG)) k_hist<K, NT_BIG * IT_BIG><<<grid, block, 0, s>>>(k, n, nb, g, pass * 8, hist);
    else k_hist<K, NT_HUGE * IT_HUGE><<<grid, block, 0, s>>>(k, n, nb, g, pass * 8, hist);
    COL_LAUNCH_OK();
    return COL_OK;
}

template <typename K, int VB, int IT, int NT>
int launch_scatter_one(hipStream_t s, const K *ki, K *ko, const void *vals, void *vals_out, uint64_t n, u32 nb, int shift,
                       const u32 *offsets) {
    dim3 grid(nb), block(NT);
    if constexpr (sizeof(K) == 4 && (VB == 0 || VB == 4)) {
        if (g_radix_dbg) {
            const size_t dyn = (g_radix_dbg & 1024) ? 18432 : (g_radix_dbg & 512) ? 4608 : 0;
            k_scatter<K, VB, IT, NT, true><<<grid, block, dyn, s>>>(ki, ko, vals, vals_out, n, nb, shift, offsets, DiagOn{g_radix_dbg});
            COL_LAUNCH_OK();
            return COL_OK;
        }
    }
    k_scatter<K, VB, IT, NT, false><<<grid, block, 0, s>>>(ki, ko, vals, vals_out, n, nb, shift, offsets, DiagOff{});
    COL_LAUNCH_OK();
    return COL_OK;
}

template <typename K, int IT, int NT>
int launch_scatter_it(hipStream_t s, const void *keys, void *keys_out, const void *vals, void *vals_out,
                      uint64_t n, int vb, int shift, const u32 *offsets) {
    const u32 nb = (u32)col_ceil_div(n, NT * IT);
    const K *ki = (const K *)keys;
    K *ko = (K *)keys_out;
    if (!vals || !vals_out) vb = 0;
    switch (vb) {
    case 0: return launch_scatter_one<K, 0, IT, NT>(s, ki, ko, nullptr, nullptr, n, nb, shift, offsets);
    case 4: return launch_scatter_one<K, 4, IT, NT>(s, ki, ko, vals, vals_out, n, nb, shift, offsets);
    case 8: return launch_scatter_one<K, 8, IT, NT>(s, ki, ko, vals, vals_out, n, nb, shift, offsets);
    case 16: return launch_scatter_one<K, 16, IT, NT>(s, ki, ko, vals, vals_out, n, nb, shift, offsets);
    case 32: return launch_scatter_one<K, 32, IT, NT>(s, ki, ko, vals, vals_out, n, nb, shift, offsets);
    default: return COL_EINVAL;
    }
}

template <typename K>
int launch_scatter(hipStream_t s, const void *keys, void *keys_out, const void *vals, void *vals_out,
                   uint64_t n, int vb, int shift, const u32 *offsets) {
    if (!vals || !vals_out) vb = 0;
    const u32 tile = tile_for(n, (int)sizeof(K), vb);
    if (tile == (u32)(NT_SMALL * IT_SMALL))
        return launch_scatter_it<K, IT_SMALL, NT_SMALL>(s, keys, keys_out, vals, vals_out, n, vb, shift, offsets);
    if (tile == (u32)(NT_MID * IT_BIG))
        return launch_scatter_it<K, IT_BIG, NT_MID>(s, keys, keys_out, vals, vals_out, n, vb, shift, offsets);
    if constexpr (sizeof(K) == 4) {
        if (tile == (u32)(NT_HUGE * IT_HUGE)) {
            constexpr uint64_t T = NT_HUGE * IT_HUGE;
            const u32 nb = (u32)col_ceil_div(n, T), nfull = (u32)(n / T);
            if (nfull) {
                k_scatter_huge<false><<<dim3(nfull), dim3(NT_HUGE), 0, s>>>((const u32 *)keys, (u32 *)keys_out, n, nb, 0, shift, offsets);
                COL_LAUNCH_OK();
            }
            if (nb > nfull) {
                k_scatter_huge<true><<<dim3(1), dim3(NT_HUGE), 0, s>>>((const u32 *)keys, (u32 *)keys_out, n, nb, nfull, shift, offsets);
                COL_LAUNCH_OK();
            }
            return COL_OK;
        }
        if (g_radix_wide_block && (vb == 0 || vb == 4 || vb == 8))
            return launch_scatter_it<K, IT_BIG / 2, NT_BIG * 2>(s, keys, keys_out, vals, vals_out, n, vb, shift, offsets);
        return launch_scatter_it<K, IT_BIG, NT_BIG>(s, keys, keys_out, vals, vals_out, n, vb, shift, offsets);
    }
    return COL_EINVAL;
}

inline bool native_value(int val_bytes) { return val_bytes == 0 || val_bytes == 4 || val_bytes == 8 || val_bytes == 16 || val_bytes == 32; }
inline bool wide_value(int val_bytes) { return val_bytes == 1 || val_bytes == 2 || val_bytes == 64 || val_bytes == 128; }
inline bool bad_sizes(uint64_t n, int key_bytes, int val_bytes) {
    if (key_bytes != 4 && key_bytes != 8) return true;
    if (!native_value(val_bytes)) return true;
    return n >= 0xFFFFFFFFull;
}

__global__ __launch_bounds__(256) void k_iota(u32 *__restrict__ out, uint64_t n) {
    const uint64_t i = (uint64_t)blockIdx.x * 256 + threadIdx.x;
    if (i < n) out[i] = (u32)i;
}
template <typename N>
__global__ __launch_bounds__(256) void k_widen(const N *__restrict__ in, u32 *__restrict__ out, uint64_t n) {
    const uint64_t i = (uint64_t)blockIdx.x * 256 + threadIdx.x;
    if (i < n) out[i] = (u32)in[i];
}
template <typename N>
__global__ __launch_bounds__(256) void k_narrow(const u32 *__restrict__ in, N *__restrict__ out, uint64_t n) {
    const uint64_t i = (uint64_t)blockIdx.x * 256 + threadIdx.x;
    if (i < n) out[i] = (N)in[i];
}
inline bool narrow_key(int key_bytes) { return key_bytes == 1 || key_bytes == 2; }
template <typename X, int CH>
__global__ __launch_bounds__(256) void k_gather_chunks(const X *__restrict__ in, const u32 *__restrict__ idx, X *__restrict__ out, uint64_t n) {
    const uint64_t t = (uint64_t)blockIdx.x * 256 + threadIdx.x;
    const uint64_t i = t / CH;
    if (i >= n) return;
    const u32 c = (u32)(t % CH);
    out[i * CH + c] = in[(uint64_t)idx[i] * CH + c];
}
int gather_values(hipStream_t s, const void *in, const u32 *idx, void *out, uint64_t n, int val_bytes) {
    const int ch = val_bytes >= 16 ? val_bytes / 16 : 1;
    dim3 grid((unsigned)col_ceil_div(n * ch, 256)), block(256);
    switch (val_bytes) {
    case 1: k_gather_chunks<uint8_t, 1><<<grid, block, 0, s>>>((const uint8_t *)in, idx, (uint8_t *)out, n); break;
    case 2: k_gather_chunks<uint16_t, 1><<<grid, block, 0, s>>>((const uint16_t *)in, idx, (uint16_t *)out, n); break;
    case 64: k_gather_chunks<uint4, 4><<<grid, block, 0, s>>>((const uint4 *)in, idx, (uint4 *)out, n); break;
    case 128: k_gather_chunks<uint4, 8><<<grid, block, 0, s>>>((const uint4 *)in, idx, (uint4 *)out, n); break;
    default: return COL_EINVAL;
    }
    COL_LAUNCH_OK();
    return COL_OK;
}

__global__ __launch_bounds__(256) void k_dbg_copy(const uint4 *__restrict__ in, uint4 *__restrict__ out, uint64_t nvec) {
    const uint64_t i = (uint64_t)blockIdx.x * 256 + threadIdx.x;
    if (i < nvec) out[i] = in[i];
}
__global__ __launch_bounds__(NT_BIG) void k_dbg_tile_copy(const u32 *__restrict__ in, u32 *__restrict__ out, uint64_t half_words) {
    constexpr int TILE = NT_BIG * IT_BIG;
    __shared__ __attribute__((aligned(16))) u32 s_k[TILE], s_v[TILE];
    typedef u32 v4u __attribute__((ext_vector_type(4)));
    const u32 tid = threadIdx.x, lane = tid & 63u, w = tid >> 6;
    const u32 q = gridDim.x / 8, r = gridDim.x % 8, xcd = blockIdx.x % 8;
    const u32 b = (xcd < r ? xcd * (q + 1) : r * (q + 1) + (xcd - r) * q) + blockIdx.x / 8;
    const uint64_t base = (uint64_t)b * TILE;
    const u32 *ka = in + base + w * 1024 + lane * 4, *va = in + half_words + base + w * 1024 + lane * 4;
    v4u kq[4], vq[4];
#pragma unroll
    for (int j = 0; j < 4; j++) asm volatile("global_load_dwordx4 %0, %1, off" : "=v"(kq[j]) : "v"(ka + j * 256) : "memory");
#pragma unroll
    for (int j = 0; j < 4; j++) asm volatile("global_load_dwordx4 %0, %1, off" : "=v"(vq[j]) : "v"(va + j * 256) : "memory");
#pragma unroll
    for (int j = 0; j < 4; j++) asm volatile("s_waitcnt vmcnt(0)" : "+v"(kq[j])::"memory");
#pragma unroll
    for (int j = 0; j < 4; j++) asm volatile("s_waitcnt vmcnt(0)" : "+v"(vq[j])::"memory");
#pragma unroll
    for (int j = 0; j < 4; j++) {
        *reinterpret_cast<v4u *>(s_k + w * 1024 + j * 256 + lane * 4) = kq[j];
        *reinterpret_cast<v4u *>(s_v + w * 1024 + j * 256 + lane * 4) = vq[j];
    }
    __syncthreads();
#pragma unroll
    for (int k = 0; k < IT_BIG; k++) {
        const u32 i = k * NT_BIG + tid;
        out[base + i] = s_k[i];
        out[half_words + base + i] = s_v[i];
    }
}

}

extern "C" {

int col_debug_copy(void *stream, const void *in, void *out, uint64_t bytes, int shape) {
    if (!in || !out || bytes == 0 || bytes % (2 * NT_BIG * IT_BIG * 4) != 0) return COL_EINVAL;
    if (shape == 0) k_dbg_copy<<<dim3((unsigned)(bytes / 16 / 256)), dim3(256), 0, col_stream(stream)>>>((const uint4 *)in, (uint4 *)out, bytes / 16);
    else if (shape == 1) k_dbg_tile_copy<<<dim3((unsigned)(bytes / (2 * NT_BIG * IT_BIG * 4))), dim3(NT_BIG), 0, col_stream(stream)>>>((const u32 *)in, (u32 *)out, bytes / 8);
    else return COL_EINVAL;
    COL_LAUNCH_OK();
    return COL_OK;
}

void col_debug_radix(int mode) { g_radix_dbg = mode; }

int col_debug_radix_tile(int tile) {
    if (tile == 8193 || tile == 8194) { g_radix_wide_block = tile == 8193; return COL_OK; }
    if (tile == (16 << 20) || tile == (8 << 20)) { g_big_n = (uint64_t)tile; return COL_OK; }
    if (tile != 0 && tile != NT_SMALL * IT_SMALL && tile != NT_MID * IT_BIG && tile != NT_BIG * IT_BIG && tile != NT_HUGE * IT_HUGE) return COL_EINVAL;
    g_radix_tile_override = tile;
    return COL_OK;
}

int col_debug_radix_stamps(uint64_t *out, int reset) {
    unsigned long long h[8] = {0};
    if (out) { COL_HIP(hipMemcpyFromSymbol(h, HIP_SYMBOL(g_stamp), sizeof(h))); for (int i = 0; i < 8; i++) out[i] = h[i]; }
    if (reset) { unsigned long long z[8] = {0}; COL_HIP(hipMemcpyToSymbol(HIP_SYMBOL(g_stamp), z, sizeof(z))); }
    return COL_OK;
}

uint32_t col_radix_tile(uint64_t n, int key_bytes, int val_bytes) {
    if (narrow_key(key_bytes)) key_bytes = 4;
    return tile_for(n, key_bytes, wide_value(val_bytes) ? 4 : val_bytes);
}

size_t col_radix_scratch_bytes(uint64_t n, int key_bytes, int val_bytes) {
    if (narrow_key(key_bytes))
        return col_radix_scratch_bytes(n, 4, val_bytes) + 2 * align256((size_t)n * 4);
    if (wide_value(val_bytes))
        return col_radix_scratch_bytes(n, key_bytes, 4) + 2 * align256((size_t)n * 4);
    const size_t nb = max_tiles_upto(n, key_bytes);
    const size_t hist = align256((size_t)RDIG * nb * sizeof(u32));
    return hist + align256(col_scan_scratch_bytes((uint64_t)RDIG * nb)) + align256((size_t)n * key_bytes) +
           align256((size_t)n * val_bytes) + 256;
}

int col_radix_tile_override_active(void) { return g_radix_tile_override != 0; }

int col_radix_histogram(void *stream, const void *keys, uint64_t n, int key_bytes, int val_bytes, int pass,
                        uint32_t *hist) {
    if (bad_sizes(n, key_bytes, val_bytes) || pass < 0 || pass >= key_bytes) return COL_EINVAL;
    if (n == 0) return COL_OK;
    return key_bytes == 4 ? launch_hist<uint32_t>(col_stream(stream), keys, n, val_bytes, pass, hist)
                          : launch_hist<uint64_t>(col_stream(stream), keys, n, val_bytes, pass, hist);
}

int col_radix_scatter(void *stream, const void *keys, void *keys_out, const void *vals, void *vals_out,
                      uint64_t n, int key_bytes, int val_bytes, int pass, const uint32_t *offsets) {
    if (bad_sizes(n, key_bytes, val_bytes) || pass < 0 || pass >= key_bytes) return COL_EINVAL;
    if (n == 0) return COL_OK;
    return key_bytes == 4
               ? launch_scatter<uint32_t>(col_stream(stream), keys, keys_out, vals, vals_out, n, val_bytes, pass * 8, offsets)
               : launch_scatter<uint64_t>(col_stream(stream), keys, keys_out, vals, vals_out, n, val_bytes, pass * 8, offsets);
}

__global__ __launch_bounds__(RDIG) void k_bucket_report(const u32 *__restrict__ sorted, u32 n, u32 *word) {
    static_assert(BS_SHIFT_REPORT == 22 && RDIG == 256, "col_bucket_report_block (col_common.h) is written for this digit");
    __shared__ u32 s_start[RDIG + 1];
    col_bucket_report_block(sorted, n, word, s_start);
}

int col_radix_sort_msd(void *stream, const uint32_t *keys, uint32_t *keys_out, const uint32_t *vals, uint32_t *vals_out,
                       uint64_t n, void *scratch, uint32_t *oversize) {
    return col_radix_sort_msd_dev(stream, keys, keys_out, vals, vals_out, n, scratch, oversize, nullptr);
}

int col_radix_sort_msd_dev(void *stream, const uint32_t *keys, uint32_t *keys_out, const uint32_t *vals, uint32_t *vals_out,
                           uint64_t n, void *scratch, uint32_t *oversize, const uint32_t *n_real_dev) {
    if (n == 0) return COL_OK;
    if (!scratch || !vals || !vals_out) return COL_EINVAL;
    if (n > COL_MSD_MAX_N) return COL_EINVAL;
    const u32 tile = tile_auto(n, 4, 4);
    hipStream_t s = col_stream(stream);
    const size_t nb = col_ceil_div(n, tile);
    char *p = (char *)scratch;
    u32 *hist = (u32 *)p;              p += align256((size_t)RDIG * nb * sizeof(u32));
    void *scan_scratch = p;            p += align256(col_scan_scratch_bytes((uint64_t)RDIG * nb));
    u32 *tmp_keys = (u32 *)p;          p += align256((size_t)n * 4);
    u32 *tmp_vals = (u32 *)p;
    int rc = col_scan_u32(stream, hist, (uint64_t)RDIG * nb, scan_scratch);
    if (rc) return rc;
    if (tile == (u32)(NT_SMALL * IT_SMALL)) rc = launch_scatter_it<u32, IT_SMALL, NT_SMALL>(s, keys, tmp_keys, vals, tmp_vals, n, 4, BS_SHIFT, hist);
    else rc = launch_scatter_it<u32, IT_BIG, NT_MID>(s, keys, tmp_keys, vals, tmp_vals, n, 4, BS_SHIFT, hist);
    if (rc) return rc;
    if (n <= COL_MSD_SMALL_N)
        k_bucket_sort<8><<<dim3(RDIG), dim3(BS_NT), 0, s>>>(tmp_keys, tmp_vals, keys_out, vals_out, (u32)n, hist, (u32)nb, oversize, n_real_dev);
    else
        k_bucket_sort<16><<<dim3(RDIG), dim3(BS_NT), 0, s>>>(tmp_keys, tmp_vals, keys_out, vals_out, (u32)n, hist, (u32)nb, oversize, n_real_dev);
    COL_LAUNCH_OK();
    return COL_OK;
}

static int sort_passes(void *stream, const void *keys, void *keys_out, const void *vals, void *vals_out,
                       uint64_t n, int key_bytes, int val_bytes, void *scratch, int copy_back, int have_hist0, int passes);
int col_radix_sort_low_passes(void *stream, const uint32_t *keys, uint32_t *keys_out, const uint32_t *vals,
                              uint32_t *vals_out, uint64_t n, void *scratch, int passes) {
    if (passes < 1 || passes > 4) return COL_EINVAL;
    return sort_passes(stream, keys, keys_out, vals, vals_out, n, 4, 4, scratch, 0, 0, passes);
}

int col_radix_bucket_report(void *stream, const uint32_t *sorted_codes, uint64_t n, uint32_t *word) {
    if (!sorted_codes || !word || n == 0 || n >= 0xFFFFFFFFull) return COL_EINVAL;
    k_bucket_report<<<dim3(1), dim3(RDIG), 0, col_stream(stream)>>>(sorted_codes, (u32)n, word);
    COL_LAUNCH_OK();
    return COL_OK;
}

int col_radix_sort(void *stream, const void *keys, void *keys_out, const void *vals, void *vals_out,
                   uint64_t n, int key_bytes, int val_bytes, void *scratch, int copy_back) {
    return col_radix_sort_ex(stream, keys, keys_out, vals, vals_out, n, key_bytes, val_bytes, scratch, copy_back, 0);
}

static int sort_passes(void *stream, const void *keys, void *keys_out, const void *vals, void *vals_out,
                       uint64_t n, int key_bytes, int val_bytes, void *scratch, int copy_back, int have_hist0, int passes);

int col_radix_sort_ex(void *stream, const void *keys, void *keys_out, const void *vals, void *vals_out,
                      uint64_t n, int key_bytes, int val_bytes, void *scratch, int copy_back, int have_hist0) {
    if (!vals || !vals_out) val_bytes = 0;
    if (narrow_key(key_bytes)) {
        if (n >= 0xFFFFFFFFull || have_hist0 || !(native_value(val_bytes) || wide_value(val_bytes))) return COL_EINVAL;
        if (n == 0) return COL_OK;
        if (!scratch) return COL_ENOSCRATCH;
        hipStream_t s = col_stream(stream);
        char *q = (char *)scratch + col_radix_scratch_bytes(n, 4, val_bytes);
        u32 *wide_in = (u32 *)q, *wide_out = (u32 *)(q + align256((size_t)n * 4));
        dim3 grid((unsigned)col_ceil_div(n, 256)), block(256);
        if (key_bytes == 1) k_widen<uint8_t><<<grid, block, 0, s>>>((const uint8_t *)keys, wide_in, n);
        else k_widen<uint16_t><<<grid, block, 0, s>>>((const uint16_t *)keys, wide_in, n);
        COL_LAUNCH_OK();
        int rc;
        if (wide_value(val_bytes)) {
            char *q2 = (char *)scratch + col_radix_scratch_bytes(n, 4, 4);
            u32 *iota = (u32 *)q2, *sorted_idx = (u32 *)(q2 + align256((size_t)n * 4));
            k_iota<<<grid, block, 0, s>>>(iota, n);
            COL_LAUNCH_OK();
            if ((rc = sort_passes(stream, wide_in, wide_out, iota, sorted_idx, n, 4, 4, scratch, 0, 0, key_bytes))) return rc;
            if ((rc = gather_values(s, vals, sorted_idx, vals_out, n, val_bytes))) return rc;
        } else if ((rc = sort_passes(stream, wide_in, wide_out, vals, vals_out, n, 4, val_bytes, scratch, 0, 0, key_bytes))) return rc;
        if (key_bytes == 1) k_narrow<uint8_t><<<grid, block, 0, s>>>(wide_out, (uint8_t *)keys_out, n);
        else k_narrow<uint16_t><<<grid, block, 0, s>>>(wide_out, (uint16_t *)keys_out, n);
        COL_LAUNCH_OK();
        if (copy_back) {
            COL_HIP(hipMemcpyAsync((void *)keys, keys_out, (size_t)n * key_bytes, hipMemcpyDeviceToDevice, s));
            if (val_bytes) COL_HIP(hipMemcpyAsync((void *)vals, vals_out, (size_t)n * val_bytes, hipMemcpyDeviceToDevice, s));
        }
        return COL_OK;
    }
    return sort_passes(stream, keys, keys_out, vals, vals_out, n, key_bytes, val_bytes, scratch, copy_back, have_hist0, key_bytes);
}

static int sort_passes(void *stream, const void *keys, void *keys_out, const void *vals, void *vals_out,
                       uint64_t n, int key_bytes, int val_bytes, void *scratch, int copy_back, int have_hist0, int passes) {
    if (wide_value(val_bytes)) {
        if (n >= 0xFFFFFFFFull || (key_bytes != 4 && key_bytes != 8)) return COL_EINVAL;
        if (n == 0) return COL_OK;
        if (!scratch) return COL_ENOSCRATCH;
        hipStream_t s = col_stream(stream);
        char *q = (char *)scratch + col_radix_scratch_bytes(n, key_bytes, 4);
        u32 *iota = (u32 *)q, *sorted_idx = (u32 *)(q + align256((size_t)n * 4));
        k_iota<<<dim3((unsigned)col_ceil_div(n, 256)), dim3(256), 0, s>>>(iota, n);
        COL_LAUNCH_OK();
        int rc = sort_passes(stream, keys, keys_out, iota, sorted_idx, n, key_bytes, 4, scratch, 0, 0, passes);
        if (rc) return rc;
        if ((rc = gather_values(s, vals, sorted_idx, vals_out, n, val_bytes))) return rc;
        if (copy_back) {
            COL_HIP(hipMemcpyAsync((void *)keys, keys_out, (size_t)n * key_bytes, hipMemcpyDeviceToDevice, s));
            COL_HIP(hipMemcpyAsync((void *)vals, vals_out, (size_t)n * val_bytes, hipMemcpyDeviceToDevice, s));
        }
        return COL_OK;
    }
    if (bad_sizes(n, key_bytes, val_bytes)) return COL_EINVAL;
    if (n == 0) return COL_OK;
    if (!scratch) return COL_ENOSCRATCH;
    hipStream_t s = col_stream(stream);
    const size_t nb = tiles_of(n, key_bytes, val_bytes);
    char *p = (char *)scratch;
    u32 *hist = (u32 *)p;              p += align256((size_t)RDIG * nb * sizeof(u32));
    void *scan_scratch = p;            p += align256(col_scan_scratch_bytes((uint64_t)RDIG * nb));
    void *tmp_keys = p;                p += align256((size_t)n * key_bytes);
    void *tmp_vals = p;
    const void *src_k = keys, *src_v = vals;
    for (int pass = 0; pass < passes; pass++) {
        void *dst_k = ((passes - 1 - pass) & 1) ? tmp_keys : keys_out;
        void *dst_v = ((passes - 1 - pass) & 1) ? tmp_vals : vals_out;
        int rc = (pass == 0 && have_hist0) ? COL_OK : col_radix_histogram(stream, src_k, n, key_bytes, val_bytes, pass, hist);
        if (rc) return rc;
        rc = col_scan_u32(stream, hist, (uint64_t)RDIG * nb, scan_scratch);
        if (rc) return rc;
        rc = col_radix_scatter(stream, src_k, dst_k, src_v, dst_v, n, key_bytes, val_bytes, pass, hist);
        if (rc) return rc;
        src_k = dst_k;
        src_v = dst_v;
    }
    if (copy_back) {
        COL_HIP(hipMemcpyAsync((void *)keys, keys_out, (size_t)n * key_bytes, hipMemcpyDeviceToDevice, s));
        if (val_bytes) COL_HIP(hipMemcpyAsync((void *)vals, vals_out, (size_t)n * val_bytes, hipMemcpyDeviceToDevice, s));
    }
    return COL_OK;
}

int col_ref_block_sort(void *stream, void *keys, void *vals, uint64_t n, int key_bytes, int val_bytes,
                       uint32_t block, int bits, int pass, uint32_t *hist) {
    if ((key_bytes != 4 && key_bytes != 8) || block == 0 || n % block || bits < 1 || bits > 12) return COL_EINVAL;
    if (!vals) val_bytes = 0;
    if (n == 0) return COL_OK;
    const u32 nb = (u32)(n / block);
    const size_t lds = (((size_t)4 << bits) + 15 & ~(size_t)15) + (size_t)block * (key_bytes + val_bytes);
    if (lds > 64 * 1024) return COL_EINVAL;
    if (key_bytes == 4)
        k_ref_block_sort<uint32_t><<<dim3(nb), dim3(COL_WAVE), lds, col_stream(stream)>>>(
            (uint32_t *)keys, (unsigned char *)vals, block, (u32)val_bytes, bits, pass, nb, hist);
    else
        k_ref_block_sort<uint64_t><<<dim3(nb), dim3(COL_WAVE), lds, col_stream(stream)>>>(
            (uint64_t *)keys, (unsigned char *)vals, block, (u32)val_bytes, bits, pass, nb, hist);
    COL_LAUNCH_OK();
    return COL_OK;
}

int col_ref_scatter(void *stream, const void *keys, void *keys_out, const void *vals, void *vals_out,
                    uint64_t n, int key_bytes, int val_bytes, uint32_t block, int bits, int pass,
                    const uint32_t *offsets, const uint32_t *hist) {
    if ((key_bytes != 4 && key_bytes != 8) || block == 0 || n % block || bits < 1 || bits > 12) return COL_EINVAL;
    if (n == 0) return COL_OK;
    const u32 nb = (u32)(n / block);
    const size_t lds = (size_t)8 << bits;
    if (key_bytes == 4)
        k_ref_scatter<uint32_t><<<dim3(nb), dim3(COL_WAVE), lds, col_stream(stream)>>>(
            (const uint32_t *)keys, (uint32_t *)keys_out, (const unsigned char *)vals, (unsigned char *)vals_out, block,
            (u32)val_bytes, bits, pass, nb, offsets, hist);
    else
        k_ref_scatter<uint64_t><<<dim3(nb), dim3(COL_WAVE), lds, col_stream(stream)>>>(
            (const uint64_t *)keys, (uint64_t *)keys_out, (const unsigned char *)vals, (unsigned char *)vals_out, block,
            (u32)val_bytes, bits, pass, nb, offsets, hist);
    COL_LAUNCH_OK();
    return COL_OK;
}

}
```

collision_amd/csrc/reduce.hip:

```cpp
#include "col_common.h"
#include <math.h>

namespace {

constexpr int RT = 256;
constexpr int RMAX_BLOCKS = 1024;

template <typename T, int W> struct Row { T v[W]; };

template <typename T> __device__ __forceinline__ T shfl_xor_t(T v, int o) { return __shfl_xor(v, o, COL_WAVE); }

template <typename T> __device__ __forceinline__ T pos_inf();
template <> __device__ __forceinline__ float pos_inf<float>() { return INFINITY; }
template <> __device__ __forceinline__ double pos_inf<double>() { return (double)INFINITY; }
template <> __device__ __forceinline__ uint32_t pos_inf<uint32_t>() { return 0xFFFFFFFFu; }
template <> __device__ __forceinline__ int32_t pos_inf<int32_t>() { return 0x7FFFFFFF; }
template <> __device__ __forceinline__ uint64_t pos_inf<uint64_t>() { return ~0ull; }
template <> __device__ __forceinline__ int64_t pos_inf<int64_t>() { return 0x7FFFFFFFFFFFFFFFll; }
template <typename T> __device__ __forceinline__ T neg_inf();
template <> __device__ __forceinline__ float neg_inf<float>() { return -INFINITY; }
template <> __device__ __forceinline__ double neg_inf<double>() { return -(double)INFINITY; }
template <> __device__ __forceinline__ uint32_t neg_inf<uint32_t>() { return 0u; }
template <> __device__ __forceinline__ int32_t neg_inf<int32_t>() { return (int32_t)0x80000000; }
template <> __device__ __forceinline__ uint64_t neg_inf<uint64_t>() { return 0ull; }
template <> __device__ __forceinline__ int64_t neg_inf<int64_t>() { return (int64_t)0x8000000000000000ll; }

template <typename T, int W, int OP> struct Acc {
    static constexpr int N = (OP == COL_OP_MINMAX ? 2 : 1) * W;
    T a[N];
    __device__ __forceinline__ void init() {
#pragma unroll
        for (int i = 0; i < W; i++) {
            if (OP == COL_OP_MINMAX) { a[i] = pos_inf<T>(); a[W + i] = neg_inf<T>(); }
            else a[i] = (T)0;
        }
    }
    __device__ __forceinline__ void add_row(const Row<T, W> &r) {
#pragma unroll
        for (int i = 0; i < W; i++) {
            if (OP == COL_OP_MINMAX) {
                a[i] = r.v[i] < a[i] ? r.v[i] : a[i];
                a[W + i] = r.v[i] > a[W + i] ? r.v[i] : a[W + i];
            } else a[i] += r.v[i];
        }
    }
    __device__ __forceinline__ void merge(const T *o) {
#pragma unroll
        for (int i = 0; i < W; i++) {
            if (OP == COL_OP_MINMAX) {
                a[i] = o[i] < a[i] ? o[i] : a[i];
                a[W + i] = o[W + i] > a[W + i] ? o[W + i] : a[W + i];
            } else a[i] += o[i];
        }
    }
    __device__ __forceinline__ void wave_reduce() {
#pragma unroll
        for (int o = COL_WAVE / 2; o > 0; o >>= 1) {
            T t[N];
#pragma unroll
            for (int i = 0; i < N; i++) t[i] = shfl_xor_t(a[i], o);
            merge(t);
        }
    }
};

template <typename T, int W, int OP>
__device__ __forceinline__ void block_fold(Acc<T, W, OP> &acc, T *out) {
    constexpr int N = Acc<T, W, OP>::N;
    __shared__ T s[(RT / COL_WAVE) * N];
    acc.wave_reduce();
    const u32 lane = lane_id(), w = threadIdx.x / COL_WAVE;
    if (lane == 0) {
#pragma unroll
        for (int i = 0; i < N; i++) s[w * N + i] = acc.a[i];
    }
    __syncthreads();
    if (threadIdx.x == 0) {
        for (int k = 1; k < RT / COL_WAVE; k++) acc.merge(&s[k * N]);
#pragma unroll
        for (int i = 0; i < N; i++) out[i] = acc.a[i];
    }
}

template <typename T, int W, int OP>
__global__ __launch_bounds__(RT) void k_reduce1(const Row<T, W> *__restrict__ rows, uint64_t n, T *partials) {
    Acc<T, W, OP> acc;
    acc.init();
    const uint64_t stride = (uint64_t)gridDim.x * RT;
    uint64_t i = (uint64_t)blockIdx.x * RT + threadIdx.x;
    if constexpr (OP == COL_OP_MINMAX && W == 4) {
        for (; i + 7 * stride < n; i += 8 * stride) {
            Row<T, W> r[8];
#pragma unroll
            for (int u = 0; u < 8; u++) r[u] = rows[i + u * stride];
#pragma unroll
            for (int u = 0; u < 8; u++) acc.add_row(r[u]);
        }
    }
    for (; i + 3 * stride < n; i += 4 * stride) {
        Row<T, W> r0 = rows[i], r1 = rows[i + stride], r2 = rows[i + 2 * stride], r3 = rows[i + 3 * stride];
        acc.add_row(r0); acc.add_row(r1); acc.add_row(r2); acc.add_row(r3);
    }
    for (; i < n; i += stride) acc.add_row(rows[i]);
    block_fold<T, W, OP>(acc, partials + (size_t)blockIdx.x * Acc<T, W, OP>::N);
}

template <typename T>
__global__ __launch_bounds__(RT) void k_minmax4_dev(const Row<T, 4> *__restrict__ rows, const u32 *__restrict__ n_dev, u32 n_max,
                                                    T *partials) {
    Acc<T, 4, COL_OP_MINMAX> acc;
    acc.init();
    const uint64_t n = min(*n_dev, n_max);
    const uint64_t stride = (uint64_t)gridDim.x * RT;
    uint64_t i = (uint64_t)blockIdx.x * RT + threadIdx.x;
    for (; i + 7 * stride < n; i += 8 * stride) {
        Row<T, 4> r[8];
#pragma unroll
        for (int u = 0; u < 8; u++) r[u] = rows[i + u * stride];
#pragma unroll
        for (int u = 0; u < 8; u++) acc.add_row(r[u]);
    }
    for (; i + 3 * stride < n; i += 4 * stride) {
        Row<T, 4> r0 = rows[i], r1 = rows[i + stride], r2 = rows[i + 2 * stride], r3 = rows[i + 3 * stride];
        acc.add_row(r0); acc.add_row(r1); acc.add_row(r2); acc.add_row(r3);
    }
    for (; i < n; i += stride) acc.add_row(rows[i]);
    block_fold<T, 4, COL_OP_MINMAX>(acc, partials + (size_t)blockIdx.x * Acc<T, 4, COL_OP_MINMAX>::N);
}

template <typename T, int W, int OP>
__global__ __launch_bounds__(RT) void k_reduce2(const T *partials, uint32_t nparts, T *out) {
    constexpr int N = Acc<T, W, OP>::N;
    Acc<T, W, OP> acc;
    acc.init();
    for (uint32_t i = threadIdx.x; i < nparts; i += RT) acc.merge(partials + (size_t)i * N);
    block_fold<T, W, OP>(acc, out);
}

template <typename T, int W, int OP>
int launch(void *stream, const void *values, uint64_t n, void *scratch, void *out) {
    uint64_t blocks = col_ceil_div(n, (uint64_t)RT * 4);
    if (blocks > RMAX_BLOCKS) blocks = RMAX_BLOCKS;
    if (blocks == 0) blocks = 1;
    k_reduce1<T, W, OP><<<dim3((unsigned)blocks), dim3(RT), 0, col_stream(stream)>>>(
        (const Row<T, W> *)values, n, (T *)scratch);
    COL_LAUNCH_OK();
    k_reduce2<T, W, OP><<<dim3(1), dim3(RT), 0, col_stream(stream)>>>((const T *)scratch, (uint32_t)blocks, (T *)out);
    COL_LAUNCH_OK();
    return COL_OK;
}

template <typename T, int OP>
int by_width(void *stream, const void *values, uint64_t n, int width, void *scratch, void *out) {
    switch (width) {
    case 1: return launch<T, 1, OP>(stream, values, n, scratch, out);
    case 2: return launch<T, 2, OP>(stream, values, n, scratch, out);
    case 4: return launch<T, 4, OP>(stream, values, n, scratch, out);
    case 8: return launch<T, 8, OP>(stream, values, n, scratch, out);
    case 16: return launch<T, 16, OP>(stream, values, n, scratch, out);
    default: return COL_EINVAL;
    }
}

template <typename T>
int by_op(void *stream, const void *values, uint64_t n, int width, int op, void *scratch, void *out) {
    if (op == COL_OP_MINMAX) return by_width<T, COL_OP_MINMAX>(stream, values, n, width, scratch, out);
    if (op == COL_OP_SUM) return by_width<T, COL_OP_SUM>(stream, values, n, width, scratch, out);
    return COL_EINVAL;
}

struct AccList { int n; int op[COL_REDUCE_MAX_ACC]; double init[COL_REDUCE_MAX_ACC]; long long iinit[COL_REDUCE_MAX_ACC]; int exact[COL_REDUCE_MAX_ACC]; };

template <typename T> __device__ __forceinline__ T init_value(const AccList &L, int k) {
    if (k >= L.n) return (T)0;
    const double v = L.init[k];
    if (v == (double)INFINITY) return pos_inf<T>();
    if (v == -(double)INFINITY) return neg_inf<T>();
    if constexpr (!__is_floating_point(T)) { if (L.exact[k]) return (T)(unsigned long long)L.iinit[k]; }
    return (T)v;
}
template <typename T> __device__ __forceinline__ T apply_op(int op, T a, T b) {
    switch (op) {
    case COL_ACC_MIN: return b < a ? b : a;
    case COL_ACC_MAX: return b > a ? b : a;
    case COL_ACC_MUL: return a * b;
    default: return a + b;
    }
}

template <typename T, int W>
__device__ __forceinline__ void fold_list(const AccList &L, T (&a)[COL_REDUCE_MAX_ACC][W], T *out) {
    __shared__ T s[(RT / COL_WAVE) * COL_REDUCE_MAX_ACC * W];
    const u32 lane = lane_id(), w = threadIdx.x / COL_WAVE;
    for (int k = 0; k < L.n; k++) {
#pragma unroll
        for (int o = COL_WAVE / 2; o > 0; o >>= 1) {
#pragma unroll
            for (int i = 0; i < W; i++) a[k][i] = apply_op(L.op[k], a[k][i], shfl_xor_t(a[k][i], o));
        }
        if (lane == 0) {
#pragma unroll
            for (int i = 0; i < W; i++) s[(w * COL_REDUCE_MAX_ACC + k) * W + i] = a[k][i];
        }
    }
    __syncthreads();
    if (threadIdx.x == 0) {
        for (int k = 0; k < L.n; k++) {
            for (int i = 0; i < W; i++) {
                T v = a[k][i];
                for (int ww = 1; ww < RT / COL_WAVE; ww++) v = apply_op(L.op[k], v, s[(ww * COL_REDUCE_MAX_ACC + k) * W + i]);
                out[k * W + i] = v;
            }
        }
    }
}

template <typename T, int W>
__global__ __launch_bounds__(RT) void k_reduce_list1(const Row<T, W> *__restrict__ rows, uint64_t n, AccList L, T *partials) {
    T a[COL_REDUCE_MAX_ACC][W];
    for (int k = 0; k < COL_REDUCE_MAX_ACC; k++)
#pragma unroll
        for (int i = 0; i < W; i++) a[k][i] = init_value<T>(L, k);
    const uint64_t stride = (uint64_t)gridDim.x * RT;
    for (uint64_t i = (uint64_t)blockIdx.x * RT + threadIdx.x; i < n; i += stride) {
        const Row<T, W> r = rows[i];
        for (int k = 0; k < L.n; k++)
#pragma unroll
            for (int c = 0; c < W; c++) a[k][c] = apply_op(L.op[k], a[k][c], r.v[c]);
    }
    fold_list<T, W>(L, a, partials + (size_t)blockIdx.x * L.n * W);
}

template <typename T, int W>
__global__ __launch_bounds__(RT) void k_reduce_list2(const T *partials, uint32_t nparts, AccList L, T *out) {
    T a[COL_REDUCE_MAX_ACC][W];
    for (int k = 0; k < COL_REDUCE_MAX_ACC; k++)
#pragma unroll
        for (int i = 0; i < W; i++) a[k][i] = init_value<T>(L, k);
    for (uint32_t p = threadIdx.x; p < nparts; p += RT)
        for (int k = 0; k < L.n; k++)
#pragma unroll
            for (int c = 0; c < W; c++) a[k][c] = apply_op(L.op[k], a[k][c], partials[((size_t)p * L.n + k) * W + c]);
    fold_list<T, W>(L, a, out);
}

template <typename T, int W>
int launch_list(void *stream, const void *values, uint64_t n, const AccList &L, void *scratch, void *out) {
    uint64_t blocks = col_ceil_div(n, (uint64_t)RT * 4);
    if (blocks > RMAX_BLOCKS) blocks = RMAX_BLOCKS;
    if (blocks == 0) blocks = 1;
    k_reduce_list1<T, W><<<dim3((unsigned)blocks), dim3(RT), 0, col_stream(stream)>>>((const Row<T, W> *)values, n, L, (T *)scratch);
    COL_LAUNCH_OK();
    k_reduce_list2<T, W><<<dim3(1), dim3(RT), 0, col_stream(stream)>>>((const T *)scratch, (uint32_t)blocks, L, (T *)out);
    COL_LAUNCH_OK();
    return COL_OK;
}

template <typename T>
int list_by_width(void *stream, const void *values, uint64_t n, int width, const AccList &L, void *scratch, void *out) {
    switch (width) {
    case 1: return launch_list<T, 1>(stream, values, n, L, scratch, out);
    case 2: return launch_list<T, 2>(stream, values, n, L, scratch, out);
    case 4: return launch_list<T, 4>(stream, values, n, L, scratch, out);
    case 8: return launch_list<T, 8>(stream, values, n, L, scratch, out);
    case 16: return launch_list<T, 16>(stream, values, n, L, scratch, out);
    default: return COL_EINVAL;
    }
}

}

extern "C" {

int col_minmax4_stage1(void *stream, const void *rows, uint64_t n, int coord_bytes, void *partials, uint32_t *parts) {
    uint64_t blocks = col_ceil_div(n, (uint64_t)RT * 16);
    if (blocks > COL_MINMAX_PARTS) blocks = COL_MINMAX_PARTS;
    if (blocks == 0) blocks = 1;
    *parts = (uint32_t)blocks;
    if (coord_bytes == 4)
        k_reduce1<float, 4, COL_OP_MINMAX><<<dim3((unsigned)blocks), dim3(RT), 0, col_stream(stream)>>>(
            (const Row<float, 4> *)rows, n, (float *)partials);
    else if (coord_bytes == 8)
        k_reduce1<double, 4, COL_OP_MINMAX><<<dim3((unsigned)blocks), dim3(RT), 0, col_stream(stream)>>>(
            (const Row<double, 4> *)rows, n, (double *)partials);
    else
        return COL_EINVAL;
    COL_LAUNCH_OK();
    return COL_OK;
}

int col_minmax4_stage1_dev(void *stream, const void *rows, const uint32_t *n_dev, uint32_t n_max, int coord_bytes, void *partials,
                           uint32_t *parts) {
    if (!n_dev || !partials || !parts) return COL_EINVAL;
    uint64_t blocks = col_ceil_div(n_max, (uint64_t)RT * 16);
    if (blocks > COL_MINMAX_PARTS) blocks = COL_MINMAX_PARTS;
    if (blocks == 0) blocks = 1;
    *parts = (uint32_t)blocks;
    if (coord_bytes == 4)
        k_minmax4_dev<float><<<dim3((unsigned)blocks), dim3(RT), 0, col_stream(stream)>>>((const Row<float, 4> *)rows, n_dev, n_max, (float *)partials);
    else if (coord_bytes == 8)
        k_minmax4_dev<double><<<dim3((unsigned)blocks), dim3(RT), 0, col_stream(stream)>>>((const Row<double, 4> *)rows, n_dev, n_max, (double *)partials);
    else
        return COL_EINVAL;
    COL_LAUNCH_OK();
    return COL_OK;
}

size_t col_reduce_scratch_bytes(int dtype, int width) {
    size_t eb = (dtype == COL_F32 || dtype == COL_U32 || dtype == COL_I32) ? 4 : 8;
    return (size_t)RMAX_BLOCKS * COL_REDUCE_MAX_ACC * (size_t)width * eb;
}

int col_reduce_list(void *stream, const void *values, uint64_t n, int dtype, int width, int n_acc, const int *ops,
                    const double *inits, const int64_t *int_inits, void *scratch, void *out) {
    if (!scratch) return COL_ENOSCRATCH;
    if (n_acc < 1 || n_acc > COL_REDUCE_MAX_ACC || !ops || !inits) return COL_EINVAL;
    AccList L;
    L.n = n_acc;
    for (int k = 0; k < COL_REDUCE_MAX_ACC; k++) {
        L.op[k] = k < n_acc ? ops[k] : COL_ACC_ADD;
        L.init[k] = k < n_acc ? inits[k] : 0.0;
        L.exact[k] = k < n_acc && int_inits != nullptr;
        L.iinit[k] = L.exact[k] ? (long long)int_inits[k] : 0;
        if (L.op[k] < COL_ACC_MIN || L.op[k] > COL_ACC_MUL) return COL_EINVAL;
    }
    switch (dtype) {
    case COL_F32: return list_by_width<float>(stream, values, n, width, L, scratch, out);
    case COL_F64: return list_by_width<double>(stream, values, n, width, L, scratch, out);
    case COL_U32: return list_by_width<uint32_t>(stream, values, n, width, L, scratch, out);
    case COL_I32: return list_by_width<int32_t>(stream, values, n, width, L, scratch, out);
    case COL_U64: return list_by_width<uint64_t>(stream, values, n, width, L, scratch, out);
    case COL_I64: return list_by_width<int64_t>(stream, values, n, width, L, scratch, out);
    default: return COL_EINVAL;
    }
}

int col_reduce(void *stream, const void *values, uint64_t n, int dtype, int width, int op,
               void *scratch, void *out) {
    if (!scratch) return COL_ENOSCRATCH;
    switch (dtype) {
    case COL_F32: return by_op<float>(stream, values, n, width, op, scratch, out);
    case COL_F64: return by_op<double>(stream, values, n, width, op, scratch, out);
    case COL_U32: return by_op<uint32_t>(stream, values, n, width, op, scratch, out);
    case COL_I32: return by_op<int32_t>(stream, values, n, width, op, scratch, out);
    case COL_U64: return by_op<uint64_t>(stream, values, n, width, op, scratch, out);
    case COL_I64: return by_op<int64_t>(stream, values, n, width, op, scratch, out);
    default: return COL_EINVAL;
    }
}

}
```

Before: 6412 M spheres/s.

## Fuse MSD sort histogram scan into Morton and scatter; compute cross bounds directly

The Morton kernel now writes its per-tile digit histograms block-major and atomically accumulates grouped digit sums into a buffer zeroed by the min/max reduction kernel. The MSD scatter kernel derives its own bucket offsets from the group sums and the preceding tiles' histograms, which removes the separate histogram scan launch. Separately, the LBVH cross-chunk bound computation for small n now merges chunk totals straight from the first table, using per-thread, per-wave or per-block strategies by span, instead of building the multi-level tables. This cuts kernel launches and passes at the cost of more redundant loads per scatter block and atomics in the Morton kernel.

```diff
diff --git a/collision_amd/csrc/bvh.hip b/collision_amd/csrc/bvh.hip
--- a/collision_amd/csrc/bvh.hip
+++ b/collision_amd/csrc/bvh.hip
@@ -1249,7 +1249,8 @@
     return 256  + col_reduce_scratch_bytes(coord_bytes == 8 ? COL_F64 : COL_F32, 4) +
            col_radix_scratch_bytes(padded, 4, 4) + col_lbvh_scratch_bytes(n, coord_bytes) +
            (size_t)n * 4 * coord_bytes  + sizeof(ChunkHdr) + 256  + 1024 +
-           8 * ((size_t)n / 64 + 1) + 256 ;
+           8 * ((size_t)n / 64 + 1) + 256  +
+           256 + col_radix_msd_fused_bytes() ;
 }
 
 int col_collide(void *stream, const void *coords, const void *radii, uint32_t n, uint32_t padded, int coord_bytes,
@@ -1301,7 +1302,9 @@
     p = (char *)(((uintptr_t)p + 255) & ~(uintptr_t)255);
     void *packed = p;          p += (size_t)n * 4 * coord_bytes;
     p = (char *)(((uintptr_t)p + 255) & ~(uintptr_t)255);
-    void *chunk_hdr = p;
+    void *chunk_hdr = p;       p += sizeof(ChunkHdr) + 256 + 8 * ((size_t)n / 64 + 1) + 256;
+    p = (char *)(((uintptr_t)p + 255) & ~(uintptr_t)255);
+    uint32_t *msd_fused = (uint32_t *)p;
     const bool chunked = (sort_plan & COL_TRAVERSE_CHUNKED) != 0;
     sort_plan &= 1;
     uint32_t *publish = oversize ? oversize + 2 : nullptr;
@@ -1310,14 +1313,17 @@
     const uint32_t tile = col_radix_tile(padded, 4, 4);
     if (tile == 1024 || tile == 4096 || tile == 8192) {
         const bool msd = sort_plan == COL_SORT_MSD && padded <= COL_MSD_MAX_N;
+        const uint32_t nsums = msd ? (uint32_t)(col_radix_msd_fused_bytes() / sizeof(uint32_t)) : 0u;
+        if (msd && col_ceil_div(padded, tile) > (uint64_t)COL_MSD_GROUP * COL_MSD_GROUPS) return COL_EINVAL;
         if (!partials) {
-            if ((rc = col_minmax4_stage1(stream, coords, n, coord_bytes, red_scratch, &parts))) return rc;
+            if ((rc = col_minmax4_stage1_zero(stream, coords, n, coord_bytes, red_scratch, &parts, msd_fused, nsums))) return rc;
             partials = red_scratch;
-        }
+        } else if (msd)
+            COL_HIP(hipMemsetAsync(msd_fused, 0, nsums * sizeof(uint32_t), s));
         if ((rc = col_morton_tile(stream, coords, radii, partials, parts, n, padded, coord_bytes, codes0, ids0, packed,
                                   counter, (uint32_t *)sort_scratch, tile, (uint32_t)col_ceil_div(padded, tile), msd ? 22 : 0,
-                                  publish, n_dev))) return rc;
-        if (msd) rc = col_radix_sort_msd_dev(stream, codes0, codes1, ids0, ids1, padded, sort_scratch, oversize, n_dev);
+                                  publish, n_dev, msd ? msd_fused : nullptr))) return rc;
+        if (msd) rc = col_radix_sort_msd_fused(stream, codes0, codes1, ids0, ids1, padded, sort_scratch, oversize, n_dev, msd_fused);
         else rc = col_radix_sort_ex(stream, codes0, codes1, ids0, ids1, padded, 4, 4, sort_scratch, 0, 1);
         if (rc) return rc;
         if (!msd && oversize && padded <= COL_MSD_MAX_N) report_word = oversize + 1;
diff --git a/collision_amd/csrc/col_common.h b/collision_amd/csrc/col_common.h
--- a/collision_amd/csrc/col_common.h
+++ b/collision_amd/csrc/col_common.h
@@ -44,7 +44,14 @@
 extern "C" int col_morton_tile(void *stream, const void *coords, const void *radii, const void *partials, uint32_t parts,
                                uint32_t n, uint32_t padded, int coord_bytes, uint32_t *codes, uint32_t *ids, void *packed,
                                uint32_t *zero_word, uint32_t *hist0, uint32_t tile, uint32_t nblocks, int hist_shift,
-                               uint32_t *publish, const uint32_t *n_dev);
+                               uint32_t *publish, const uint32_t *n_dev, uint32_t *gsum);
+#define COL_MSD_GROUP 32u
+#define COL_MSD_GROUPS 32u
+extern "C" int col_minmax4_stage1_zero(void *stream, const void *rows, uint64_t n, int coord_bytes, void *partials, uint32_t *parts,
+                                       uint32_t *zero, uint32_t nzero);
+extern "C" size_t col_radix_msd_fused_bytes(void);
+extern "C" int col_radix_sort_msd_fused(void *stream, const uint32_t *keys, uint32_t *keys_out, const uint32_t *vals, uint32_t *vals_out,
+                                        uint64_t n, void *scratch, uint32_t *oversize, const uint32_t *n_real_dev, uint32_t *fused);
 extern "C" int col_radix_sort_ex(void *stream, const void *keys, void *keys_out, const void *vals, void *vals_out,
                                  uint64_t n, int key_bytes, int val_bytes, void *scratch, int copy_back, int have_hist0);
 
diff --git a/collision_amd/csrc/lbvh.hip b/collision_amd/csrc/lbvh.hip
--- a/collision_amd/csrc/lbvh.hip
+++ b/collision_amd/csrc/lbvh.hip
@@ -788,7 +788,111 @@
     row[4] = box.hi[0]; row[5] = box.hi[1]; row[6] = box.hi[2];
 }
 
+constexpr u32 CROSS_SHORT = 8;
+constexpr u32 CROSS_LIST = (256 / CROSS_CAP) * C;
+#ifndef COL_CROSS_DIRECT_MAX_N
+#define COL_CROSS_DIRECT_MAX_N COL_MSD_MAX_N
+#endif
+constexpr u32 CROSS_DIRECT_MAX_CHUNKS = COL_CROSS_DIRECT_MAX_N / C;
+
+__device__ __forceinline__ uint64_t chunk_total_at(u32 e) { return (uint64_t)(e / C) * (LV * C) + e % C; }
+
 template <typename T>
+__device__ __forceinline__ void cross_store(T *__restrict__ bounds, u32 i, const Box<T> &box) {
+    T *row = bounds + 8ull * i;
+    row[0] = box.lo[0]; row[1] = box.lo[1]; row[2] = box.lo[2];
+    row[4] = box.hi[0]; row[5] = box.hi[1]; row[6] = box.hi[2];
+}
+
+template <typename T> struct CrossU { static constexpr u32 U = sizeof(T) == 4 ? 16 : 8; };
+constexpr u32 CROSS_MID_U = 8, CROSS_MID = COL_WAVE * CROSS_MID_U;
+struct CrossLds {
+    uint2 list[CROSS_LIST];
+    u32 nmid, nhuge;
+    double part[256 / COL_WAVE][6];
+};
+
+template <typename T>
+__device__ __forceinline__ void cross_direct(T *__restrict__ bounds, const u32 *__restrict__ other_end, const T *__restrict__ partial,
+                                             const T *__restrict__ tab0, u32 i, CrossLds &lds) {
+    const u32 j = other_end[i];
+    const u32 first = min(i, j), last = max(i, j);
+    const u32 a = first / C + 1, b = last / C;
+    if (b < a) return;
+    if (b - a > CROSS_MID) { lds.list[CROSS_LIST - 1 - atomicAdd(&lds.nhuge, 1u)] = make_uint2(i, j); return; }
+    if (b - a > CROSS_SHORT) { lds.list[atomicAdd(&lds.nmid, 1u)] = make_uint2(i, j); return; }
+    Box<T> box = box_load(partial, first);
+    box_merge(box, box_load(partial, last));
+    if (b > a) {
+        Box<T> v[CROSS_SHORT];
+#pragma unroll
+        for (u32 k = 0; k < CROSS_SHORT; k++) v[k] = box_load(tab0, chunk_total_at(min(a + k, b - 1)));
+#pragma unroll
+        for (u32 k = 0; k < CROSS_SHORT; k++) box_merge(box, v[k]);
+    }
+    cross_store(bounds, i, box);
+}
+
+template <typename T> __device__ __forceinline__ void box_wave_union(Box<T> &box) {
+#pragma unroll
+    for (int o = COL_WAVE / 2; o > 0; o >>= 1) {
+        Box<T> r;
+#pragma unroll
+        for (int k = 0; k < 3; k++) { r.lo[k] = __shfl_xor(box.lo[k], o, COL_WAVE); r.hi[k] = __shfl_xor(box.hi[k], o, COL_WAVE); }
+        box_merge(box, r);
+    }
+}
+
+template <typename T, u32 U>
+__device__ __forceinline__ void cross_batch(const T *__restrict__ tab0, u32 e0, u32 stride, u32 b, Box<T> &box) {
+    Box<T> v[U];
+#pragma unroll
+    for (u32 k = 0; k < U; k++) v[k] = box_load(tab0, chunk_total_at(min(e0 + stride * k, b - 1)));
+#pragma unroll
+    for (u32 k = 0; k < U; k++) box_merge(box, v[k]);
+}
+
+template <typename T>
+__device__ __forceinline__ void cross_direct_wave(T *__restrict__ bounds, const T *__restrict__ partial,
+                                                  const T *__restrict__ tab0, uint2 ij, u32 lane) {
+    const u32 first = min(ij.x, ij.y), last = max(ij.x, ij.y);
+    const u32 a = first / C + 1, b = last / C;
+    Box<T> box = box_load(partial, first);
+    box_merge(box, box_load(partial, last));
+    cross_batch<T, CROSS_MID_U>(tab0, a + lane, COL_WAVE, b, box);
+    box_wave_union(box);
+    if (lane == 0) cross_store(bounds, ij.x, box);
+}
+
+template <typename T>
+__device__ __forceinline__ void cross_direct_block(T *__restrict__ bounds, const T *__restrict__ partial,
+                                                   const T *__restrict__ tab0, uint2 ij, CrossLds &lds) {
+    constexpr u32 U = CrossU<T>::U;
+    const u32 tid = threadIdx.x, lane = tid % COL_WAVE, w = tid / COL_WAVE;
+    const u32 first = min(ij.x, ij.y), last = max(ij.x, ij.y);
+    const u32 a = first / C + 1, b = last / C;
+    Box<T> box = box_load(partial, first);
+    box_merge(box, box_load(partial, last));
+    for (u32 e0 = a; e0 < b; e0 += 256 * U) cross_batch<T, U>(tab0, e0 + tid, 256, b, box);
+    box_wave_union(box);
+    if (lane == 0) {
+#pragma unroll
+        for (int k = 0; k < 3; k++) { lds.part[w][k] = (double)box.lo[k]; lds.part[w][3 + k] = (double)box.hi[k]; }
+    }
+    __syncthreads();
+    if (tid == 0) {
+        for (u32 ww = 1; ww < 256 / COL_WAVE; ww++) {
+            Box<T> o;
+#pragma unroll
+            for (int k = 0; k < 3; k++) { o.lo[k] = (T)lds.part[ww][k]; o.hi[k] = (T)lds.part[ww][3 + k]; }
+            box_merge(box, o);
+        }
+        cross_store(bounds, ij.x, box);
+    }
+    __syncthreads();
+}
+
+template <typename T, bool DIRECT = false>
 __global__ __launch_bounds__(256) void k_cross(T *__restrict__ bounds, const u32 *__restrict__ other_end,
                                                const T *__restrict__ partial, const u32 *__restrict__ cross, Tabs tabs, u32 n,
                                                u32 nchunks, int lin, u32 *__restrict__ zero8, const u32 *__restrict__ n_dev,
@@ -802,6 +906,29 @@
     const u32 t = blockIdx.x * 256 + threadIdx.x;
     if (zero8 && t < nzero) zero8[t] = 0;
     const u32 chunk = t / CROSS_CAP, slot = t % CROSS_CAP;
+    if constexpr (DIRECT) {
+        __shared__ CrossLds lds;
+        const T *tab0 = (const T *)tabs.t[0];
+        if (threadIdx.x == 0) { lds.nmid = 0; lds.nhuge = 0; }
+        __syncthreads();
+        if (chunk < nchunks) {
+            if (cross[(uint64_t)chunk * CROSS_CAP + CROSS_CAP - 1] == CROSS_DENSE) {
+                for (u32 k = slot; k < (u32)C; k += CROSS_CAP) {
+                    const u32 i = chunk * C + k;
+                    if (i + 1 < n) cross_direct(bounds, other_end, partial, tab0, i, lds);
+                }
+            } else {
+                const u32 i = cross[(uint64_t)chunk * CROSS_CAP + slot];
+                if (i != END) cross_direct(bounds, other_end, partial, tab0, i, lds);
+            }
+        }
+        __syncthreads();
+        const u32 nhuge = lds.nhuge, nmid = lds.nmid;
+        for (u32 q = 0; q < nhuge; q++) cross_direct_block(bounds, partial, tab0, lds.list[CROSS_LIST - 1 - q], lds);
+        for (u32 q = threadIdx.x / COL_WAVE; q < nmid; q += 256 / COL_WAVE)
+            cross_direct_wave(bounds, partial, tab0, lds.list[q], threadIdx.x % COL_WAVE);
+        return;
+    }
     if (chunk >= nchunks) return;
     if (cross[(uint64_t)chunk * CROSS_CAP + CROSS_CAP - 1] == CROSS_DENSE) {
         for (u32 k = slot; k < (u32)C; k += CROSS_CAP) {
@@ -815,6 +942,8 @@
 }
 
 int g_dbg = 0;
+constexpr int DBG_TABLES = 32768;
+constexpr int DBG_PLAIN = 1024 | 2048 | 4096 | 8192 | 16384 | DBG_TABLES;
 float g_block_k = 3.0f;
 inline size_t align256(size_t x) { return (x + 255) & ~(size_t)255; }
 
@@ -853,9 +982,9 @@
     for (int h = 0; h < 3; h++) tabs.t[h] = scratch + L.tab[h];
     const u32 nchunks = L.count[0];
     bool ordered_by_chunk = false;
-    if (g_dbg & ~(1024 | 2048 | 4096 | 8192 | 16384))
+    if (g_dbg & ~DBG_PLAIN)
         k_chunk<T, true, int64_t><<<dim3(nchunks), dim3(C), 0, s>>>(codes, ids, coords, radii, packed, nodes, bounds, other_end, partial, cross,
-                                                                    (T *)tabs.t[0], n, (T)g_block_k, n_dev, ChunkDiagOn{g_dbg & ~(1024 | 2048 | 4096 | 8192 | 16384)});
+                                                                    (T *)tabs.t[0], n, (T)g_block_k, n_dev, ChunkDiagOn{g_dbg & ~DBG_PLAIN});
     else if (n < (1u << 30) && (g_dbg & 8192))
         k_chunk<T, false, int32_t, true, true><<<dim3(nchunks), dim3(C), 0, s>>>(codes, ids, coords, radii, packed, nodes, bounds, other_end, partial, cross,
                                                                                  (T *)tabs.t[0], n, (T)g_block_k, n_dev, ChunkDiagOff{});
@@ -885,6 +1014,14 @@
         if (zero8) COL_HIP(hipMemsetAsync(zero8, 0, nzero * sizeof(u32), s));
         return COL_OK;
     }
+    const unsigned cross_blocks = (unsigned)col_ceil_div((uint64_t)nchunks * CROSS_CAP, 256);
+    const dim3 cross_grid(cross_blocks + (walk_order && !ordered_by_chunk ? 8u * COL_ORDER_SLICES : 0u));
+    if (nchunks <= CROSS_DIRECT_MAX_CHUNKS && !(g_dbg & DBG_TABLES)) {
+        k_cross<T, true><<<cross_grid, dim3(256), 0, s>>>(bounds, other_end, partial, cross, tabs, n, nchunks, -1, zero8,
+                                                          n_dev, walk_order, cross_blocks, order_mode, nzero);
+        COL_LAUNCH_OK();
+        return COL_OK;
+    }
     int lin = -1;
     for (int h = 0; h < 3; h++) {
         if (h > 0 && L.count[h] <= LIN) { lin = h; break; }
@@ -893,9 +1030,8 @@
         COL_LAUNCH_OK();
         if (groups < 2) break;
     }
-    const unsigned cross_blocks = (unsigned)col_ceil_div((uint64_t)nchunks * CROSS_CAP, 256);
-    k_cross<T><<<dim3(cross_blocks + (walk_order && !ordered_by_chunk ? 8u * COL_ORDER_SLICES : 0u)), dim3(256), 0, s>>>(bounds, other_end, partial, cross, tabs, n, nchunks, lin, zero8,
-                                                                                                          n_dev, walk_order, cross_blocks, order_mode, nzero);
+    k_cross<T><<<cross_grid, dim3(256), 0, s>>>(bounds, other_end, partial, cross, tabs, n, nchunks, lin, zero8,
+                                                n_dev, walk_order, cross_blocks, order_mode, nzero);
     COL_LAUNCH_OK();
     return COL_OK;
 }
diff --git a/collision_amd/csrc/morton.hip b/collision_amd/csrc/morton.hip
--- a/collision_amd/csrc/morton.hip
+++ b/collision_amd/csrc/morton.hip
@@ -45,7 +45,7 @@
                                                      u32 *__restrict__ ids, const T *__restrict__ radii,
                                                      Vec4<T> *__restrict__ packed, u32 *__restrict__ zero_word,
                                                      u32 *__restrict__ hist0, u32 nblocks, int hist_shift, u32 *publish,
-                                                     const u32 *__restrict__ n_dev) {
+                                                     const u32 *__restrict__ n_dev, u32 *__restrict__ gsum) {
     constexpr int TILE = NT * MT_ROWS * HALVES, NW = NT / 64;
     const u32 n = count_of(n_bound, n_dev);
     __shared__ T s_fold[NW][8];
@@ -138,23 +138,31 @@
         }
     }
     __syncthreads();
+    if (gsum) {
+        if (tid < 256) {
+            const u32 c = s_hist[tid];
+            hist0[(uint64_t)blockIdx.x * 256 + tid] = c;
+            if (c) atomicAdd(&gsum[(blockIdx.x / COL_MSD_GROUP) * 256 + tid], c);
+        }
+        return;
+    }
     if (tid < 256) hist0[(uint64_t)tid * nblocks + blockIdx.x] = s_hist[tid];
 }
 
 template <typename T>
 int launch_morton_tile(hipStream_t s, u32 tile, const void *coords, const void *radii, const void *partials, uint32_t parts,
                        uint32_t n, uint32_t padded, uint32_t *codes, uint32_t *ids, void *packed, uint32_t *zero_word,
-                       uint32_t *hist0, uint32_t nblocks, int hist_shift, uint32_t *publish, const uint32_t *n_dev) {
+                       uint32_t *hist0, uint32_t nblocks, int hist_shift, uint32_t *publish, const uint32_t *n_dev, uint32_t *gsum) {
     dim3 grid(nblocks);
     if (tile == 1024)
         k_morton_tile<T, 256, 1><<<grid, dim3(256), 0, s>>>((const Vec4<T> *)coords, (const T *)partials, parts, n, padded, codes, ids,
-                                                             (const T *)radii, (Vec4<T> *)packed, zero_word, hist0, nblocks, hist_shift, publish, n_dev);
+                                                             (const T *)radii, (Vec4<T> *)packed, zero_word, hist0, nblocks, hist_shift, publish, n_dev, gsum);
     else if (tile == 4096)
         k_morton_tile<T, 1024, 1><<<grid, dim3(1024), 0, s>>>((const Vec4<T> *)coords, (const T *)partials, parts, n, padded, codes, ids,
-                                                               (const T *)radii, (Vec4<T> *)packed, zero_word, hist0, nblocks, hist_shift, publish, n_dev);
+                                                               (const T *)radii, (Vec4<T> *)packed, zero_word, hist0, nblocks, hist_shift, publish, n_dev, gsum);
     else
         k_morton_tile<T, 1024, 2><<<grid, dim3(1024), 0, s>>>((const Vec4<T> *)coords, (const T *)partials, parts, n, padded, codes, ids,
-                                                               (const T *)radii, (Vec4<T> *)packed, zero_word, hist0, nblocks, hist_shift, publish, n_dev);
+                                                               (const T *)radii, (Vec4<T> *)packed, zero_word, hist0, nblocks, hist_shift, publish, n_dev, gsum);
     COL_LAUNCH_OK();
     return COL_OK;
 }
@@ -166,7 +174,7 @@
 int col_morton_tile(void *stream, const void *coords, const void *radii, const void *partials, uint32_t parts,
                     uint32_t n, uint32_t padded, int coord_bytes, uint32_t *codes, uint32_t *ids, void *packed,
                     uint32_t *zero_word, uint32_t *hist0, uint32_t tile, uint32_t nblocks, int hist_shift, uint32_t *publish,
-                    const uint32_t *n_dev) {
+                    const uint32_t *n_dev, uint32_t *gsum) {
     if (padded < n || parts == 0 || !hist0 || hist_shift < 0 || hist_shift > 24) return COL_EINVAL;
     if (tile != 1024 && tile != 4096 && tile != 8192) return COL_EINVAL;
     if (padded == 0) return COL_OK;
@@ -174,10 +182,10 @@
     if (nblocks != (uint32_t)col_ceil_div(padded, tile)) return COL_EINVAL;
     if (coord_bytes == 4)
         return launch_morton_tile<float>(col_stream(stream), tile, coords, radii, partials, parts, n, padded, codes, ids, packed,
-                                         zero_word, hist0, nblocks, hist_shift, publish, n_dev);
+                                         zero_word, hist0, nblocks, hist_shift, publish, n_dev, gsum);
     if (coord_bytes == 8)
         return launch_morton_tile<double>(col_stream(stream), tile, coords, radii, partials, parts, n, padded, codes, ids, packed,
-                                          zero_word, hist0, nblocks, hist_shift, publish, n_dev);
+                                          zero_word, hist0, nblocks, hist_shift, publish, n_dev, gsum);
     return COL_EINVAL;
 }
 
diff --git a/collision_amd/csrc/radix.hip b/collision_amd/csrc/radix.hip
--- a/collision_amd/csrc/radix.hip
+++ b/collision_amd/csrc/radix.hip
@@ -146,11 +146,20 @@
 
 template <bool NARROW> struct CntType { typedef u32 T; };
 template <> struct CntType<true> { typedef uint16_t T; };
-template <typename K, int VB, int IT, int NT, bool DIAG>
+constexpr int MSD_GROUP = COL_MSD_GROUP, MSD_GROUPS = COL_MSD_GROUPS;
+static_assert((uint64_t)NT_SMALL * IT_SMALL * MSD_GROUP * MSD_GROUPS >= (1u << 20) && (uint64_t)NT_MID * IT_BIG * MSD_GROUP * MSD_GROUPS >= COL_MSD_MAX_N,
+              "the group sums cover every tile count of the MSD plan");
+struct FusedOff {};
+struct FusedOn { const u32 *gsum; u32 *starts; };
+template <bool FUSED> struct FusedArg { typedef FusedOff T; };
+template <> struct FusedArg<true> { typedef FusedOn T; };
+template <typename K, int VB, int IT, int NT, bool DIAG, bool FUSED = false>
 __global__ __launch_bounds__(NT) void k_scatter(const K *__restrict__ keys_in, K *__restrict__ keys_out,
                                                 const void *__restrict__ vals_in_, void *__restrict__ vals_out_,
                                                 uint64_t n, u32 nblocks, int shift,
-                                                const u32 *__restrict__ offsets, typename DiagArg<DIAG>::T diag) {
+                                                const u32 *__restrict__ offsets, typename DiagArg<DIAG>::T diag,
+                                                typename FusedArg<FUSED>::T fused = {}) {
+    static_assert(!FUSED || (NT == RDIG && !DIAG), "the fused form: one thread per digit, production instance only");
     const int dbg = diag_mode(diag);
     constexpr int TILE = NT * IT;
     constexpr int NW = NT / COL_WAVE;
@@ -182,7 +191,9 @@
     unsigned long long t_prev = (DIAG && (dbg & 32)) ? __builtin_amdgcn_s_memtime() : 0ull;
     (void)t_prev;
     if (DIAG && (dbg & (1 << 27))) __builtin_amdgcn_s_setprio(3);
-    const u32 my_offset = tid < RDIG ? offsets[(uint64_t)tid * nblocks + b] : 0u;
+    u32 my_offset = 0;
+    u32 fused_below = 0, fused_total = 0;
+    if constexpr (!FUSED) my_offset = tid < RDIG ? offsets[(uint64_t)tid * nblocks + b] : 0u;
     for (u32 i = tid; i < NW * RDIG; i += NT) (&s_cnt[0][0])[i] = (CNT)0;
 
     const u32 wbase = w * (COL_WAVE * IT) + lane;
@@ -196,6 +207,14 @@
     V *vstage = s_vals + w * (COL_WAVE * IT);
     const bool full = valid == (u32)TILE && !(dbg & 8);
     if (full) {
+        u32 gs[FUSED ? MSD_GROUPS : 1], hs[FUSED ? MSD_GROUP - 1 : 1];
+        if constexpr (FUSED) {
+            const u32 b0 = b & ~(u32)(MSD_GROUP - 1);
+#pragma unroll
+            for (int g = 0; g < MSD_GROUPS; g++) gs[g] = (fused.gsum + g * RDIG)[tid];
+#pragma unroll
+            for (int t = 0; t < MSD_GROUP - 1; t++) hs[t] = (offsets + (size_t)min(b0 + t, nblocks - 1) * RDIG)[tid];
+        }
         K *stage = s_keys + w * (COL_WAVE * IT);
         const K *src = keys_in + tile_base + w * (COL_WAVE * IT);
         const V *vsrc = vals_in + tile_base + w * (COL_WAVE * IT);
@@ -227,7 +246,34 @@
         __builtin_amdgcn_wave_barrier();
 #pragma unroll
         for (int k = 0; k < IT; k++) key[k] = stage[k * COL_WAVE + lane];
+        if constexpr (FUSED) {
+            const u32 gb = b / MSD_GROUP, tb = b % MSD_GROUP;
+#pragma unroll
+            for (int g = 0; g < MSD_GROUPS; g++) {
+                asm volatile("" : "+v"(gs[g]));
+                fused_total += gs[g];
+                fused_below += (u32)g < gb ? gs[g] : 0u;
+            }
+#pragma unroll
+            for (int t = 0; t < MSD_GROUP - 1; t++) {
+                asm volatile("" : "+v"(hs[t]));
+                fused_below += (u32)t < tb ? hs[t] : 0u;
+            }
+            asm volatile("" : "+v"(fused_below), "+v"(fused_total));
+        }
     } else {
+        if constexpr (FUSED) {
+            const u32 gb = b / MSD_GROUP, b0 = b & ~(u32)(MSD_GROUP - 1);
+#pragma unroll 1
+            for (u32 g = 0; g < (u32)MSD_GROUPS; g++) {
+                const u32 v = (fused.gsum + g * RDIG)[tid];
+                fused_total += v;
+                fused_below += g < gb ? v : 0u;
+            }
+#pragma unroll 1
+            for (u32 t = b0; t < b; t++) fused_below += (offsets + (size_t)t * RDIG)[tid];
+            asm volatile("" : "+v"(fused_below), "+v"(fused_total)::"memory");
+        }
 #pragma unroll
         for (int k = 0; k < IT; k++) {
             const u32 li = wbase + k * COL_WAVE;
@@ -306,6 +352,12 @@
         }
     } else
     {
+        if constexpr (FUSED) {
+            u32 all;
+            const u32 bucket_start = block_excl_scan<NT>(fused_total, s_ws, &all);
+            my_offset = bucket_start + fused_below;
+            if (b == 0) fused.starts[tid] = bucket_start;
+        }
         u32 c[NW], tot = 0;
         if (tid < RDIG) {
 #pragma unroll
@@ -1000,6 +1052,36 @@
         k_bucket_sort<8><<<dim3(RDIG), dim3(BS_NT), 0, s>>>(tmp_keys, tmp_vals, keys_out, vals_out, (u32)n, hist, (u32)nb, oversize, n_real_dev);
     else
         k_bucket_sort<16><<<dim3(RDIG), dim3(BS_NT), 0, s>>>(tmp_keys, tmp_vals, keys_out, vals_out, (u32)n, hist, (u32)nb, oversize, n_real_dev);
+    COL_LAUNCH_OK();
+    return COL_OK;
+}
+
+size_t col_radix_msd_fused_bytes(void) { return (size_t)(MSD_GROUPS + 1) * RDIG * sizeof(u32); }
+int col_radix_sort_msd_fused(void *stream, const uint32_t *keys, uint32_t *keys_out, const uint32_t *vals, uint32_t *vals_out,
+                             uint64_t n, void *scratch, uint32_t *oversize, const uint32_t *n_real_dev, uint32_t *fused) {
+    if (n == 0) return COL_OK;
+    if (!scratch || !vals || !vals_out || !fused) return COL_EINVAL;
+    if (n > COL_MSD_MAX_N) return COL_EINVAL;
+    const u32 tile = tile_auto(n, 4, 4);
+    hipStream_t s = col_stream(stream);
+    const size_t nb = col_ceil_div(n, tile);
+    if (nb > (size_t)MSD_GROUP * MSD_GROUPS) return COL_EINVAL;
+    char *p = (char *)scratch;
+    const u32 *counts = (const u32 *)p; p += align256((size_t)RDIG * nb * sizeof(u32));
+    p += align256(col_scan_scratch_bytes((uint64_t)RDIG * nb));
+    u32 *tmp_keys = (u32 *)p;          p += align256((size_t)n * 4);
+    u32 *tmp_vals = (u32 *)p;
+    u32 *starts = fused + MSD_GROUPS * RDIG;
+    const FusedOn f{fused, starts};
+    if (tile == (u32)(NT_SMALL * IT_SMALL))
+        k_scatter<u32, 4, IT_SMALL, NT_SMALL, false, true><<<dim3((unsigned)nb), dim3(NT_SMALL), 0, s>>>(keys, tmp_keys, vals, tmp_vals, n, (u32)nb, BS_SHIFT, counts, DiagOff{}, f);
+    else
+        k_scatter<u32, 4, IT_BIG, NT_MID, false, true><<<dim3((unsigned)nb), dim3(NT_MID), 0, s>>>(keys, tmp_keys, vals, tmp_vals, n, (u32)nb, BS_SHIFT, counts, DiagOff{}, f);
+    COL_LAUNCH_OK();
+    if (n <= COL_MSD_SMALL_N)
+        k_bucket_sort<8><<<dim3(RDIG), dim3(BS_NT), 0, s>>>(tmp_keys, tmp_vals, keys_out, vals_out, (u32)n, starts, 1u, oversize, n_real_dev);
+    else
+        k_bucket_sort<16><<<dim3(RDIG), dim3(BS_NT), 0, s>>>(tmp_keys, tmp_vals, keys_out, vals_out, (u32)n, starts, 1u, oversize, n_real_dev);
     COL_LAUNCH_OK();
     return COL_OK;
 }
diff --git a/collision_amd/csrc/reduce.hip b/collision_amd/csrc/reduce.hip
--- a/collision_amd/csrc/reduce.hip
+++ b/collision_amd/csrc/reduce.hip
@@ -83,7 +83,9 @@
 }
 
 template <typename T, int W, int OP>
-__global__ __launch_bounds__(RT) void k_reduce1(const Row<T, W> *__restrict__ rows, uint64_t n, T *partials) {
+__global__ __launch_bounds__(RT) void k_reduce1(const Row<T, W> *__restrict__ rows, uint64_t n, T *partials,
+                                                 u32 *__restrict__ zero = nullptr, u32 nzero = 0) {
+    for (u32 z = blockIdx.x * RT + threadIdx.x; z < nzero; z += gridDim.x * RT) zero[z] = 0;
     Acc<T, W, OP> acc;
     acc.init();
     const uint64_t stride = (uint64_t)gridDim.x * RT;
@@ -273,16 +275,22 @@
 extern "C" {
 
 int col_minmax4_stage1(void *stream, const void *rows, uint64_t n, int coord_bytes, void *partials, uint32_t *parts) {
+    return col_minmax4_stage1_zero(stream, rows, n, coord_bytes, partials, parts, nullptr, 0);
+}
+
+int col_minmax4_stage1_zero(void *stream, const void *rows, uint64_t n, int coord_bytes, void *partials, uint32_t *parts,
+                            uint32_t *zero, uint32_t nzero) {
+    if (!zero) nzero = 0;
     uint64_t blocks = col_ceil_div(n, (uint64_t)RT * 16);
     if (blocks > COL_MINMAX_PARTS) blocks = COL_MINMAX_PARTS;
     if (blocks == 0) blocks = 1;
     *parts = (uint32_t)blocks;
     if (coord_bytes == 4)
         k_reduce1<float, 4, COL_OP_MINMAX><<<dim3((unsigned)blocks), dim3(RT), 0, col_stream(stream)>>>(
-            (const Row<float, 4> *)rows, n, (float *)partials);
+            (const Row<float, 4> *)rows, n, (float *)partials, zero, nzero);
     else if (coord_bytes == 8)
         k_reduce1<double, 4, COL_OP_MINMAX><<<dim3((unsigned)blocks), dim3(RT), 0, col_stream(stream)>>>(
-            (const Row<double, 4> *)rows, n, (double *)partials);
+            (const Row<double, 4> *)rows, n, (double *)partials, zero, nzero);
     else
         return COL_EINVAL;
     COL_LAUNCH_OK();
```

Result: faster. 6643 M spheres/s, median of 6 (+3.6%).
